# reedrosenbluth/LASS

Hardware: AMD Instinct MI355X
Metric: clips/sec (10s@16kHz) (higher is better)
Workload: dtype f32; 1 GPU; ResUNet30 separate() fp32, batch=16/GPU, 10s@16kHz clips, fixed precomputed condition embedding, seeded random-init weights (BASELINE configs[1]); samples_per_clip=160000, parallelism=clip-sharded x1

## Files before the change

### include/lass_hip.h

```cpp
#ifndef LASS_HIP_H
#define LASS_HIP_H

#include <stddef.h>
#include <stdint.h>

#ifdef __cplusplus
extern "C" {
#endif

typedef struct lass_ctx lass_ctx;

#define LASS_OK 0
#define LASS_ERR_ARG (-1)
#define LASS_ERR_HIP (-2)
#define LASS_ERR_STATE (-3)
#define LASS_ERR_WORKSPACE (-4)

#define LASS_F32 0
#define LASS_I64 1

#define LASS_COMPUTE_F32 0
#define LASS_COMPUTE_BF16 1
#define LASS_COMPUTE_BF16X3 2

int lass_version(void);

int lass_create(lass_ctx** out, int device_id);
int lass_create_multistft(lass_ctx** out, int device_id, int n_fft, int n_windows, const int* win_lengths,
                          int mask_window);
int lass_destroy(lass_ctx* ctx);

const char* lass_last_error(const lass_ctx* ctx);

int lass_set_param(lass_ctx* ctx, const char* name, const void* data, const int64_t* shape, int ndim, int dtype);

int lass_finalize(lass_ctx* ctx, int compute_mode);

int lass_workspace_bytes(const lass_ctx* ctx, int B, int L, size_t* bytes);

int lass_separate(lass_ctx* ctx, const float* mixture, const float* condition, float* out, int B, int L,
                  void* workspace, size_t workspace_bytes, void* stream);

int lass_graph_stats(const lass_ctx* ctx, long* captures, long* replays);
int lass_set_graph_replay(lass_ctx* ctx, int enabled);
int lass_set_wino4_splits(lass_ctx* ctx, int splits);

int lass_separate_components(lass_ctx* ctx, const float* const* mag, const float* cos_mask, const float* sin_mask,
                             const float* condition, float* out, int B, int L, void* workspace, size_t workspace_bytes,
                             void* stream);


int lass_stft_magphase(lass_ctx* ctx, const float* wav, int B, int L, float* mag, float* cos_out, float* sin_out,
                       float* real_out, float* imag_out, void* stream);

int lass_multi_stft(lass_ctx* ctx, const float* wav, int B, int L, int hop, int n_windows, const int* win_lengths,
                    float* const* mag, float* const* cos_out, float* const* sin_out, void* stream);

int lass_stft_components(lass_ctx* ctx, const float* wav, int B, int L, int n_fft, int hop, int n_windows,
                         const int* win_lengths, float* const* mag, float* const* cos_out, float* const* sin_out,
                         void* stream);

int lass_istft(lass_ctx* ctx, const float* real, const float* imag, int B, int T, int L, float* wav,
               float* frames_ws, void* stream);
int lass_istft_nfft(lass_ctx* ctx, const float* real, const float* imag, int B, int T, int L, int n_fft, int win_length,
                    float* wav, void* stream);

int lass_film(lass_ctx* ctx, const float* condition, int B, float* shift, void* stream);
int lass_film_width(const lass_ctx* ctx);
int lass_film_offset(const lass_ctx* ctx, const char* site);
int lass_film_raw(lass_ctx* ctx, const float* condition, int B, float* film, void* stream);

int lass_convblock(lass_ctx* ctx, const char* prefix, const float* x, int B, int H, int W, const float* shift,
                   float* y, float* scratch, void* stream);

int lass_encoder_block(lass_ctx* ctx, const char* name, const float* x, int B, int H, int W, const float* shift, float* y,
                       float* pool, float* scratch, void* stream);

int lass_front_end(lass_ctx* ctx, const float* wav, int B, int L, float* mag, float* cos_out, float* sin_out, float* x0,
                   void* stream);

int lass_workspace_tensor(const lass_ctx* ctx, int B, int L, const char* name, size_t* offset, int64_t shape[4],
                          int64_t strides[4]);

int lass_upconv(lass_ctx* ctx, const char* name, const float* x, int B, int h, int w, const float* shift, float* y,
                void* stream);

int lass_mask_apply(lass_ctx* ctx, const float* x12, const float* mag, const float* cos_in, const float* sin_in,
                    int B, int T, int Tpad, float* out_real, float* out_imag, void* stream);

int lass_sdr_stats(lass_ctx* ctx, const float* ref, const float* est, int B, int L, double* stats, void* stream);

int lass_mix_at_snr(lass_ctx* ctx, float* source, const float* noise, const float* snr_db, float* mixture, int B, int L,
                    double* scratch, void* stream);

#define LASS_WAV_PCM16 0
#define LASS_WAV_PCM32 1
#define LASS_WAV_F32 2
#define LASS_RESAMPLE_MAX_TAPS 16383
#define LASS_RESAMPLE_MAX_TABLE 20480
#define LASS_RESAMPLE_MAX_RATIO 65536
int lass_decode_resample(lass_ctx* ctx, const void* raw, int64_t row_stride_bytes, int B, int frames, int channels, int encoding,
                         int up, int down, const float* taps, int n_taps, float* out, int L_out, void* stream);

int lass_segment_mix(lass_ctx* ctx, const float* waveforms, int B, int L, const int* mix_num, const float* comp_db, int max_comp,
                     const float* noise_db, float* mixture, float* segment, double* scratch, void* stream);


typedef struct lass_text_ctx lass_text_ctx;

int lass_text_create(lass_text_ctx** out, int device_id);
int lass_text_destroy(lass_text_ctx* ctx);
const char* lass_text_last_error(const lass_text_ctx* ctx);
int lass_text_set_param(lass_text_ctx* ctx, const char* name, const void* data, const int64_t* shape, int ndim);
int lass_text_finalize(lass_text_ctx* ctx);
int lass_text_layers(const lass_text_ctx* ctx);
int lass_text_workspace_bytes(const lass_text_ctx* ctx, int N, int S, size_t* bytes);
int lass_text_encode(lass_text_ctx* ctx, const int64_t* input_ids, const int64_t* attention_mask, int N, int S,
                     float* out, float* pooler_out, void* workspace, size_t workspace_bytes, void* stream);


typedef struct lass_audioq_ctx lass_audioq_ctx;

typedef struct lass_audioq_taps {
    float* wave48k;
    float* logmel;
    float* tokens;
    float* stage[4];
    float* embedding;
} lass_audioq_taps;

int lass_audioq_create(lass_audioq_ctx** out, int device_id);
int lass_audioq_destroy(lass_audioq_ctx* ctx);
const char* lass_audioq_last_error(const lass_audioq_ctx* ctx);
int lass_audioq_set_param(lass_audioq_ctx* ctx, const char* name, const void* data, const int64_t* shape, int ndim);
int lass_audioq_finalize(lass_audioq_ctx* ctx);
int lass_audioq_stages(const lass_audioq_ctx* ctx);
int lass_audioq_workspace_bytes(const lass_audioq_ctx* ctx, int B, size_t* bytes);
int lass_audioq_encode_wave48k(lass_audioq_ctx* ctx, const float* wave, const int* lengths, int B, int L, float* out,
                               const lass_audioq_taps* taps, void* workspace, size_t workspace_bytes, void* stream);
int lass_audioq_encode_wave32k(lass_audioq_ctx* ctx, const float* wave, const int* lengths, int B, int L, float* out,
                               const lass_audioq_taps* taps, void* workspace, size_t workspace_bytes, void* stream);


int lass_set_profiling(lass_ctx* ctx, int enabled);
int lass_profile_count(const lass_ctx* ctx);
int lass_profile_get(lass_ctx* ctx, int i, const char** name, double* ms, int* launches);
int lass_profile_reset(lass_ctx* ctx);

#ifdef __cplusplus
}
#endif
#endif
```

### lass_amd/_lib.py

```python
from __future__ import annotations

import ctypes
import os
from ctypes import POINTER, c_char_p, c_double, c_int, c_int64, c_long, c_size_t, c_void_p

_HERE = os.path.dirname(os.path.abspath(__file__))
LIB_PATH = os.environ.get("LASS_HIP_LIB") or os.path.join(_HERE, "csrc", "liblass_hip.so")

_lib = None

SYMBOLS = [
    ("lass_version", c_int, []),
    ("lass_create", c_int, [POINTER(c_void_p), c_int]),
    ("lass_create_multistft", c_int, [POINTER(c_void_p), c_int, c_int, c_int, POINTER(c_int), c_int]),
    ("lass_destroy", c_int, [c_void_p]),
    ("lass_last_error", c_char_p, [c_void_p]),
    ("lass_set_param", c_int, [c_void_p, c_char_p, c_void_p, POINTER(c_int64), c_int, c_int]),
    ("lass_finalize", c_int, [c_void_p, c_int]),
    ("lass_workspace_bytes", c_int, [c_void_p, c_int, c_int, POINTER(c_size_t)]),
    ("lass_separate", c_int, [c_void_p, c_void_p, c_void_p, c_void_p, c_int, c_int, c_void_p, c_size_t, c_void_p]),
    ("lass_stft_magphase", c_int, [c_void_p, c_void_p, c_int, c_int, c_void_p, c_void_p, c_void_p, c_void_p,
                                   c_void_p, c_void_p]),
    ("lass_mix_at_snr", c_int, [c_void_p, c_void_p, c_void_p, c_void_p, c_void_p, c_int, c_int, c_void_p, c_void_p]),
    ("lass_decode_resample", c_int, [c_void_p, c_void_p, c_int64, c_int, c_int, c_int, c_int, c_int, c_int, c_void_p, c_int,
                                     c_void_p, c_int, c_void_p]),
    ("lass_segment_mix", c_int, [c_void_p, c_void_p, c_int, c_int, c_void_p, c_void_p, c_int, c_void_p, c_void_p, c_void_p,
                                 c_void_p, c_void_p]),
    ("lass_multi_stft", c_int, [c_void_p, c_void_p, c_int, c_int, c_int, c_int, POINTER(c_int), POINTER(c_void_p),
                                POINTER(c_void_p), POINTER(c_void_p), c_void_p]),
    ("lass_graph_stats", c_int, [c_void_p, POINTER(c_long), POINTER(c_long)]),
    ("lass_set_graph_replay", c_int, [c_void_p, c_int]),
    ("lass_set_wino4_splits", c_int, [c_void_p, c_int]),
    ("lass_separate_components", c_int, [c_void_p, POINTER(c_void_p), c_void_p, c_void_p, c_void_p, c_void_p, c_int,
                                         c_int, c_void_p, c_size_t, c_void_p]),
    ("lass_stft_components", c_int, [c_void_p, c_void_p, c_int, c_int, c_int, c_int, c_int, POINTER(c_int),
                                     POINTER(c_void_p), POINTER(c_void_p), POINTER(c_void_p), c_void_p]),
    ("lass_istft_nfft", c_int, [c_void_p, c_void_p, c_void_p, c_int, c_int, c_int, c_int, c_int, c_void_p, c_void_p]),
    ("lass_istft", c_int, [c_void_p, c_void_p, c_void_p, c_int, c_int, c_int, c_void_p, c_void_p, c_void_p]),
    ("lass_film", c_int, [c_void_p, c_void_p, c_int, c_void_p, c_void_p]),
    ("lass_film_width", c_int, [c_void_p]),
    ("lass_film_offset", c_int, [c_void_p, c_char_p]),
    ("lass_film_raw", c_int, [c_void_p, c_void_p, c_int, c_void_p, c_void_p]),
    ("lass_convblock", c_int, [c_void_p, c_char_p, c_void_p, c_int, c_int, c_int, c_void_p, c_void_p, c_void_p,
                               c_void_p]),
    ("lass_encoder_block", c_int, [c_void_p, c_char_p, c_void_p, c_int, c_int, c_int, c_void_p, c_void_p, c_void_p,
                                   c_void_p, c_void_p]),
    ("lass_front_end", c_int, [c_void_p, c_void_p, c_int, c_int, c_void_p, c_void_p, c_void_p, c_void_p, c_void_p]),
    ("lass_workspace_tensor", c_int, [c_void_p, c_int, c_int, c_char_p, POINTER(c_size_t), POINTER(c_int64),
                                      POINTER(c_int64)]),
    ("lass_upconv", c_int, [c_void_p, c_char_p, c_void_p, c_int, c_int, c_int, c_void_p, c_void_p, c_void_p]),
    ("lass_mask_apply", c_int, [c_void_p, c_void_p, c_void_p, c_void_p, c_void_p, c_int, c_int, c_int, c_void_p,
                                c_void_p, c_void_p]),
    ("lass_sdr_stats", c_int, [c_void_p, c_void_p, c_void_p, c_int, c_int, c_void_p, c_void_p]),
    ("lass_text_create", c_int, [POINTER(c_void_p), c_int]),
    ("lass_text_destroy", c_int, [c_void_p]),
    ("lass_text_last_error", c_char_p, [c_void_p]),
    ("lass_text_set_param", c_int, [c_void_p, c_char_p, c_void_p, POINTER(c_int64), c_int]),
    ("lass_text_finalize", c_int, [c_void_p]),
    ("lass_text_layers", c_int, [c_void_p]),
    ("lass_text_workspace_bytes", c_int, [c_void_p, c_int, c_int, POINTER(c_size_t)]),
    ("lass_text_encode", c_int, [c_void_p, c_void_p, c_void_p, c_int, c_int, c_void_p, c_void_p, c_void_p, c_size_t,
                                 c_void_p]),
    ("lass_audioq_create", c_int, [POINTER(c_void_p), c_int]),
    ("lass_audioq_destroy", c_int, [c_void_p]),
    ("lass_audioq_last_error", c_char_p, [c_void_p]),
    ("lass_audioq_set_param", c_int, [c_void_p, c_char_p, c_void_p, POINTER(c_int64), c_int]),
    ("lass_audioq_finalize", c_int, [c_void_p]),
    ("lass_audioq_stages", c_int, [c_void_p]),
    ("lass_audioq_workspace_bytes", c_int, [c_void_p, c_int, POINTER(c_size_t)]),
    ("lass_audioq_encode_wave48k", c_int, [c_void_p, c_void_p, POINTER(c_int), c_int, c_int, c_void_p, c_void_p, c_void_p,
                                           c_size_t, c_void_p]),
    ("lass_audioq_encode_wave32k", c_int, [c_void_p, c_void_p, POINTER(c_int), c_int, c_int, c_void_p, c_void_p, c_void_p,
                                           c_size_t, c_void_p]),
    ("lass_set_profiling", c_int, [c_void_p, c_int]),
    ("lass_profile_count", c_int, [c_void_p]),
    ("lass_profile_get", c_int, [c_void_p, c_int, POINTER(c_char_p), POINTER(c_double), POINTER(c_int)]),
    ("lass_profile_reset", c_int, [c_void_p]),
]


class LassError(RuntimeError):
    pass


def load():
    global _lib
    if _lib is not None:
        return _lib
    import torch

    if not os.path.exists(LIB_PATH):
        raise LassError(
            f"{LIB_PATH} is missing - build it with `python -c 'import __graft_entry__ as g; g.build()'` "
            "(hipcc --offload-arch=gfx950).  lass_amd has no CPU fallback.")
    lib = ctypes.CDLL(LIB_PATH, mode=ctypes.RTLD_GLOBAL)
    for name, res, args in SYMBOLS:
        fn = getattr(lib, name)
        fn.restype = res
        fn.argtypes = args
    _lib = lib
    return lib


def check(ctx, rc: int, what: str):
    if rc < 0:
        msg = load().lass_last_error(ctx)
        raise LassError(f"{what} failed ({rc}): {msg.decode() if msg else '?'}")
    return rc
```

### lass_amd/csrc/api.hip

```cpp
#include <hip/hip_runtime.h>

#include <algorithm>
#include <cmath>
#include <cstdio>
#include <cstdlib>
#include <cstring>
#include <map>
#include <string>
#include <vector>

#include "../../include/lass_hip.h"
#include "kernels.h"

namespace {

struct EncSpec { const char* name; int cin, cout, dh, dw; };
struct DecSpec { const char* name; int cin, cout, uh, uw; };
const EncSpec kEnc[7] = {{"encoder_block1", 32, 32, 2, 2},   {"encoder_block2", 32, 64, 2, 2},
                         {"encoder_block3", 64, 128, 2, 2},  {"encoder_block4", 128, 256, 2, 2},
                         {"encoder_block5", 256, 384, 2, 2}, {"encoder_block6", 384, 384, 1, 2},
                         {"conv_block7a", 384, 384, 1, 1}};
const DecSpec kDec[6] = {{"decoder_block1", 384, 384, 1, 2}, {"decoder_block2", 384, 384, 2, 2},
                         {"decoder_block3", 384, 256, 2, 2}, {"decoder_block4", 256, 128, 2, 2},
                         {"decoder_block5", 128, 64, 2, 2},  {"decoder_block6", 64, 32, 2, 2}};
constexpr int kPreCh = 32;
constexpr float kBnEps = 1e-5f;
constexpr int kMaxBranches = LASS_MAX_STFT_WINDOWS;

struct Raw {
    float* d = nullptr;
    std::vector<int64_t> shape;
    size_t n = 0;
};

struct Site {
    std::string film;
    std::string bn;
    int C = 0;
    int off = 0;
};

struct ResBlock {
    std::string prefix;
    int cin = 0, cout = 0;
    int width = 0;
    int s1 = -1, s2 = -1;
    float *w1 = nullptr, *w2 = nullptr, *wsc = nullptr;
    float *u1 = nullptr, *u2 = nullptr, *usc = nullptr;
    float *u1f = nullptr, *u2f = nullptr;
    void *b1 = nullptr, *b2 = nullptr, *bsc16 = nullptr;
    void *b1l = nullptr, *b2l = nullptr, *bscl = nullptr;
    const float* bsc = nullptr;
};

struct ProfEntry {
    const char* name;
    double ms = 0;
    int launches = 0;
};

thread_local std::string g_create_err;

}

struct Geometry {
    int variant = 0;
    int nbr = 1;
    int wins[kMaxBranches] = {1024, 0, 0, 0};
    int nfft = 1024, nbins = 513, fcrop = 512;
    int mask_br = 0;
    int magphase_sem = 0;
};

struct lass_ctx {
    int device = 0;
    std::string err;
    Geometry g;
    EncSpec E[7];
    DecSpec D[6];
    int dec_cat[6] = {0};
    std::string pre_name[kMaxBranches];
    std::map<std::string, Raw> raw;
    bool finalized = false;
    float2* tw2k = nullptr;
    std::vector<Site> sites;
    std::map<std::string, int> site_idx;
    int n_shift = 0;
    float *film_W = nullptr, *film_b = nullptr, *bn_scale = nullptr, *bn_base = nullptr;
    float *bn0_s = nullptr, *bn0_h = nullptr;
    std::vector<ResBlock> enc, dec;
    int dec_site[6] = {0};
    void* up16[6] = {nullptr};
    void* up16l[6] = {nullptr};
    std::vector<void*> owned;
    int compute_mode = LASS_COMPUTE_F32;
    int wino4_mincin = 32;
    int ksplit_force = 0;
    float* stage_part = nullptr;
    size_t stage_part_floats = 0;
    bool fuse_catb = true;
    bool fuse_block = true;
    bool fuse_up = true;
    void* up_sc16 = nullptr;
    bool use_graph = true;
    struct GraphKey {
        const void *mix = nullptr, *cond = nullptr, *out = nullptr, *ws = nullptr;
        int B = 0, L = 0;
        unsigned long gen = 0;
        bool operator==(const GraphKey& o) const {
            return mix == o.mix && cond == o.cond && out == o.out && ws == o.ws && B == o.B && L == o.L && gen == o.gen;
        }
    };
    struct GraphEntry {
        GraphKey key;
        hipGraphExec_t exec = nullptr;
        size_t need = 0;
        int seen = 0;
        unsigned long used = 0;
        bool split = false;
    };
    std::map<std::pair<int, int>, bool> last_split;
    static constexpr int kGraphSlots = 4;
    GraphEntry g_slots[kGraphSlots];
    unsigned long g_tick = 0;
    std::vector<hipGraphExec_t> g_retired;
    hipStream_t g_stream = nullptr;
    int split_batch = 1;
    hipStream_t s2 = nullptr;
    hipEvent_t ev_fork = nullptr, ev_join = nullptr;
    unsigned long gen = 0;
    long g_replays = 0, g_captures = 0;
    bool profiling = false;
    std::vector<ProfEntry> prof;
    std::vector<hipEvent_t> ev_pool;
    struct Pending { int cls; hipEvent_t a, b; };
    std::vector<Pending> pending;
    size_t ev_used = 0;
};

namespace {

#define HIP_TRY(ctx, expr)                                                                                     \
    do {                                                                                                       \
        hipError_t _e = (expr);                                                                                \
        if (_e != hipSuccess) {                                                                                \
            (ctx)->err = std::string(#expr) + ": " + hipGetErrorString(_e);                                     \
            return LASS_ERR_HIP;                                                                               \
        }                                                                                                      \
    } while (0)

int fail(lass_ctx* ctx, int code, const std::string& msg) {
    if (ctx) ctx->err = msg;
    return code;
}

bool starts_with(const std::string& s, const char* p) { return s.rfind(p, 0) == 0; }
bool ends_with(const std::string& s, const char* p) {
    const size_t n = strlen(p);
    return s.size() >= n && s.compare(s.size() - n, n, p) == 0;
}

std::string film_to_bn(const std::string& film) {
    std::string s = "base.";
    for (size_t i = 0; i < film.size(); ++i) {
        if (film[i] == '-' && i + 1 < film.size() && film[i + 1] == '>') {
            s += '.';
            ++i;
        } else {
            s += film[i];
        }
    }
    const size_t p = s.rfind("beta");
    s.replace(p, 4, "bn");
    return s;
}

int add_site(lass_ctx* c, const std::string& film, int C) {
    Site s;
    s.film = film;
    s.bn = film_to_bn(film);
    s.C = C;
    s.off = c->n_shift;
    c->n_shift += C;
    c->site_idx[film] = (int)c->sites.size();
    c->sites.push_back(s);
    return (int)c->sites.size() - 1;
}

const ResBlock& trunk_block(const lass_ctx* c, int i) { return c->enc[c->g.nbr - 1 + i]; }

void build_arch(lass_ctx* c) {
    const Geometry& g = c->g;
    c->sites.clear();
    c->site_idx.clear();
    c->n_shift = 0;
    c->enc.clear();
    c->dec.clear();
    for (int i = 0; i < 7; ++i) c->E[i] = kEnc[i];
    for (int i = 0; i < 6; ++i) c->D[i] = kDec[i];
    c->E[1].cin = kPreCh * g.nbr;
    for (int k = 0; k < g.nbr; ++k) {
        ResBlock rb;
        std::string film;
        if (g.variant == 0) {
            rb.prefix = "base.encoder_block1.conv_block1";
            film = "encoder_block1->conv_block1";
            c->pre_name[k] = "base.pre_conv";
        } else {
            const std::string w = std::to_string(g.wins[k]);
            rb.prefix = "base.encoder_block1s." + w + ".conv_block1";
            film = "encoder_block1s->" + w + "->conv_block1";
            c->pre_name[k] = "base.pre_convs." + w;
        }
        rb.cin = rb.cout = kPreCh;
        rb.width = g.fcrop;
        rb.s1 = add_site(c, film + "->beta1", kPreCh);
        rb.s2 = add_site(c, film + "->beta2", kPreCh);
        c->enc.push_back(rb);
    }
    for (int i = 1; i < 7; ++i) {
        const EncSpec& e = c->E[i];
        ResBlock rb;
        rb.prefix = std::string("base.") + e.name + ".conv_block1";
        rb.cin = e.cin;
        rb.cout = e.cout;
        rb.width = g.fcrop >> i;
        rb.s1 = add_site(c, std::string(e.name) + "->conv_block1->beta1", e.cin);
        rb.s2 = add_site(c, std::string(e.name) + "->conv_block1->beta2", e.cout);
        c->enc.push_back(rb);
    }
    for (int i = 0; i < 6; ++i) {
        const auto& d = c->D[i];
        const int e = 5 - i;
        c->dec_cat[i] = d.cout + c->E[e].cout * (e == 0 ? g.nbr : 1);
        c->dec_site[i] = add_site(c, std::string(d.name) + "->beta1", d.cin);
        ResBlock rb;
        rb.prefix = std::string("base.") + d.name + ".conv_block2";
        rb.cin = c->dec_cat[i];
        rb.cout = d.cout;
        rb.width = g.fcrop >> e;
        rb.s1 = add_site(c, std::string(d.name) + "->conv_block2->beta1", rb.cin);
        rb.s2 = add_site(c, std::string(d.name) + "->conv_block2->beta2", d.cout);
        c->dec.push_back(rb);
    }
}

std::vector<int64_t> expected_shape(const lass_ctx* c, const std::string& name) {
    auto bn_field = [](const std::string& n) {
        return ends_with(n, ".weight") || ends_with(n, ".bias") || ends_with(n, ".running_mean") ||
               ends_with(n, ".running_var");
    };
    if (starts_with(name, "base.bn0.") && bn_field(name)) return {c->g.nbins};
    for (int k = 0; k < c->g.nbr; ++k) {
        if (name == c->pre_name[k] + ".weight") return {kPreCh, 1, 1, 1};
        if (name == c->pre_name[k] + ".bias") return {kPreCh};
    }
    if (name == "base.after_conv.weight") return {3, kPreCh, 1, 1};
    if (name == "base.after_conv.bias") return {3};
    auto res_block = [&](const ResBlock& rb) -> std::vector<int64_t> {
        const std::string& p = rb.prefix;
        if (!starts_with(name, (p + ".").c_str())) return {};
        const std::string f = name.substr(p.size() + 1);
        if (starts_with(f, "bn1.") && bn_field(f)) return {rb.cin};
        if (starts_with(f, "bn2.") && bn_field(f)) return {rb.cout};
        if (f == "conv1.weight") return {rb.cout, rb.cin, 3, 3};
        if (f == "conv2.weight") return {rb.cout, rb.cout, 3, 3};
        if (rb.cin != rb.cout && f == "shortcut.weight") return {rb.cout, rb.cin, 1, 1};
        if (rb.cin != rb.cout && f == "shortcut.bias") return {rb.cout};
        return {};
    };
    for (const auto& rb : c->enc) {
        auto s = res_block(rb);
        if (!s.empty()) return s;
    }
    for (int i = 0; i < 6; ++i) {
        auto s = res_block(c->dec[i]);
        if (!s.empty()) return s;
        const DecSpec& d = c->D[i];
        const std::string p = std::string("base.") + d.name;
        if (name == p + ".conv1.weight") return {d.cin, d.cout, d.uh, d.uw};
        if (starts_with(name, (p + ".bn1.").c_str()) && bn_field(name)) return {d.cin};
    }
    if (starts_with(name, "film.")) {
        for (const auto& s : c->sites) {
            if (name == "film." + s.film + ".weight") return {s.C, LASS_COND};
            if (name == "film." + s.film + ".bias") return {s.C};
        }
    }
    return {};
}

bool ignorable(const std::string& name) {
    if (starts_with(name, "base.stft.") || starts_with(name, "base.istft.")) return true;
    if (ends_with(name, "num_batches_tracked")) return true;
    for (const auto& d : kDec) {
        if (starts_with(name, (std::string("base.") + d.name + ".bn2.").c_str())) return true;
        if (starts_with(name, (std::string("film.") + d.name + "->beta2.").c_str())) return true;
    }
    return false;
}

const float* rawp(const lass_ctx* c, const std::string& name) {
    auto it = c->raw.find(name);
    return it == c->raw.end() ? nullptr : it->second.d;
}

template <typename T>
int dev_alloc(lass_ctx* c, T** p, size_t count) {
    void* v = nullptr;
    HIP_TRY(c, hipMalloc(&v, count * sizeof(T)));
    c->owned.push_back(v);
    *p = (T*)v;
    return 0;
}

void free_owned(lass_ctx* c) {
    for (void* p : c->owned) (void)hipFree(p);
    c->owned.clear();
}

enum ProfClass { P_STFT = 0, P_FILM, P_PRECONV, P_CONV3X3, P_TCONV, P_POOL, P_MASK, P_ISTFT, P_COUNT };
const char* kProfNames[P_COUNT] = {"stft_magphase", "film", "pre_conv", "conv3x3_mfma", "tconv_mfma",
                                   "avg_pool",      "mask_apply", "istft"};

constexpr size_t kProfPairs = 512;

struct ProfScope {
    lass_ctx* c;
    hipStream_t s;
    int cls;
    hipEvent_t b = nullptr;
    bool on = false;
    ProfScope(lass_ctx* ctx, hipStream_t st, int k) : c(ctx), s(st), cls(k) {
        if (!c->profiling || c->ev_used + 2 > c->ev_pool.size()) return;
        hipEvent_t a = c->ev_pool[c->ev_used++];
        b = c->ev_pool[c->ev_used++];
        (void)hipEventRecord(a, s);
        c->pending.push_back({cls, a, b});
        on = true;
    }
    ~ProfScope() {
        if (on) (void)hipEventRecord(b, s);
    }
};

void prof_collect(lass_ctx* c) {
    for (auto& p : c->pending) {
        float ms = 0;
        if (hipEventElapsedTime(&ms, p.a, p.b) == hipSuccess) {
            c->prof[p.cls].ms += ms;
            c->prof[p.cls].launches += 1;
        }
    }
    c->pending.clear();
    c->ev_used = 0;
}

struct CatCopies {
    void* act;
    void* raw;
    int noct;
    const float* scale;
    const float* shift;
};

struct MaskHead {
    const float* mag;
    const float* cosv;
    const float* sinv;
    float* oreal;
    float* oimag;
    int T;
    int nbins;
};

struct PreConv {
    const float* x0;
    const float* w;
    const float* b;
};

struct UpFuse {
    const void* x_act;
    int cin, h, w;
    const void* w16;
    const void* wsc16;
};

struct BlockFusions {
    float* pool_out = nullptr;
    int pool_h = 2;
    long pool_bs = 0;
    int cofs = 0;
    const PreConv* pre = nullptr;
    const MaskHead* head = nullptr;
    const CatCopies* skip_out = nullptr;
    const CatCopies* cat_in = nullptr;
    const Site* act_out = nullptr;
    const CatCopies* pool_copies = nullptr;
    const UpFuse* up = nullptr;
    float* kpart = nullptr;
};

constexpr int kWino4Splits = 4;
int wino4_splits(const lass_ctx* c, const ResBlock& rb, int B, int H, int W) {
    (void)B;
    if (c->compute_mode != LASS_COMPUTE_F32 || c->wino4_mincin <= 0 || !lass_wino4_narrow(H, W) || rb.width % 32 != 16) return 0;
    if (rb.cin < c->wino4_mincin || rb.cout < c->wino4_mincin || rb.cin % 8 != 0 || rb.cout % 32 != 0) return 0;
    return c->ksplit_force ? c->ksplit_force : kWino4Splits;
}
size_t wino4_split_floats(const ResBlock& rb, int S, int B, int H, int W) { return S > 1 ? (size_t)S * B * rb.cout * H * W : 0; }

constexpr int kShortcutGemmMinCin = 256;

int run_resblock(lass_ctx* c, const ResBlock& rb, const float* x, long x_bs, int B, int H, int W, const float* shift,
                 float* a2, float* out, long out_bs, hipStream_t st, const BlockFusions& f = BlockFusions()) {
    const PreConv* pre = f.pre;
    const CatCopies *skip_out = f.skip_out, *cat_in = f.cat_in, *pool_copies = f.pool_copies;
    const float* x0 = pre ? pre->x0 : nullptr;
    const Site& s1 = c->sites[rb.s1];
    const Site& s2 = c->sites[rb.s2];
    const long HW = (long)H * W;
    ConvArgs p;
    p.in = x; p.in_bs = x_bs; p.Cin = rb.cin; p.w = rb.w1; p.Nw = rb.cout; p.N = rb.cout;
    p.pro_scale = c->bn_scale + s1.off; p.pro_shift = shift + s1.off; p.pro_shift_bs = c->n_shift;
    p.epi_scale = c->bn_scale + s2.off; p.epi_shift = shift + s2.off; p.epi_shift_bs = c->n_shift;
    p.out = a2; p.out_bs = rb.cout * HW; p.B = B; p.H = H; p.W = W;
    if (x0) {
        p.in = x0; p.in_bs = HW;
        p.pre_w = pre->w; p.pre_b = pre->b;
    }
    p.w_wino = rb.u1; p.w_wino4 = rb.u1f;
    p.w_bf16 = rb.b1; p.w_bf16_lo = rb.b1l;
    const bool bf1 = c->compute_mode != LASS_COMPUTE_F32 && rb.b1 && rb.b2 && lass_bf16_supported(p) &&
                     (!x0 || W % 32 == 0) && rb.cout % 16 == 0 && (rb.cin == rb.cout || (rb.bsc16 && rb.cin % 16 == 0));
    void* a2_hi = a2;
    void* a2_lo = c->compute_mode == LASS_COMPUTE_BF16X3 ? (void*)((char*)a2 + (size_t)B * rb.cout * HW * 2) : nullptr;
    if (bf1) { p.out_bf16 = a2_hi; p.out_bf16_lo = a2_lo; }
    if ((skip_out || cat_in) && (!bf1 || c->compute_mode != LASS_COMPUTE_BF16))
        return fail(c, LASS_ERR_STATE, "blocked bf16 concat copies need the bf16 kernels");
    if (cat_in) p.in_bf16 = cat_in->act;
    const ConvKind k1 = x0 ? CONV1_ACT_PRE : CONV1_ACT, k2 = x0 ? CONV2_IDENT_PRE : CONV2_IDENT;
    const bool wino1 = !bf1 && rb.u1 && lass_wino_supported(p);
    const int ksplit = bf1 || x0 ? 0 : wino4_splits(c, rb, B, H, W);
    const bool w4_geom = rb.width % 32 == 0 ? !lass_wino4_narrow(H, W) : ksplit > 0;
    if (ksplit > 1) {
        if (!f.kpart) return fail(c, LASS_ERR_STATE, "split-K needs its partial workspace");
        const auto overlaps = [&](const float* a, size_t a_n, const float* b, long b_bs, long b_n) {
            return a < b + (size_t)(B - 1) * b_bs + b_n && b < a + a_n;
        };
        const size_t kn = wino4_split_floats(rb, ksplit, B, H, W);
        if (overlaps(f.kpart, kn, x, x_bs, rb.cin * HW) || overlaps(f.kpart, kn, a2, rb.cout * HW, rb.cout * HW) ||
            overlaps(f.kpart, kn, out, out_bs, rb.cout * HW))
            return fail(c, LASS_ERR_STATE, "the split-K partials must not overlap the block's input, intermediate or output");
    }
    Wino4Split sk;
    if (ksplit > 1) { sk.n = ksplit; sk.part = f.kpart; }
    auto launch_conv1 = [&]() -> int {
        ProfScope ps(c, st, P_CONV3X3);
        if (bf1)
            HIP_TRY(c, lass_launch_conv_bf16(k1, p, st));
        else if (wino1 && rb.u1f && w4_geom && lass_wino4_supported(k1, p, sk))
            HIP_TRY(c, lass_launch_wino4(k1, p, st, sk));
        else if (wino1)
            HIP_TRY(c, lass_launch_wino(k1, p, st));
        else
            HIP_TRY(c, lass_launch_conv(k1, p, st));
        return 0;
    };
    ConvArgs q;
    q.in = a2; q.in_bs = rb.cout * HW; q.Cin = rb.cout; q.w = rb.w2; q.Nw = rb.cout; q.N = rb.cout;
    q.out = out; q.out_bs = out_bs; q.B = B; q.H = H; q.W = W;
    q.pool_out = f.pool_out; q.pool_h = f.pool_h; q.pool_bs = f.pool_bs;
    q.w_wino = rb.u2; q.w2_wino = rb.usc; q.w_wino4 = w4_geom ? rb.u2f : nullptr;
    if (const MaskHead* mh = f.head) {
        q.out = nullptr;
        q.mask_w = rawp(c, "base.after_conv.weight"); q.mask_b = rawp(c, "base.after_conv.bias");
        q.mask_mag = mh->mag; q.mask_cos = mh->cosv; q.mask_sin = mh->sinv;
        q.mask_re = mh->oreal; q.mask_im = mh->oimag; q.mask_T = mh->T; q.mask_nbins = mh->nbins;
    }
    q.w_bf16 = rb.b2; q.w2_bf16 = rb.bsc16; q.w_bf16_lo = rb.b2l; q.w2_bf16_lo = rb.bscl;
    const bool bf2 = bf1;
    if (bf2) { q.in_bf16 = a2_hi; q.in_bf16_lo = a2_lo; }
    if (cat_in) q.in2_bf16 = cat_in->raw;
    if (pool_copies) {
        if (!bf2 || c->compute_mode != LASS_COMPUTE_BF16 || !f.pool_out || f.pool_h != 2)
            return fail(c, LASS_ERR_STATE, "blocked bf16 pooled copies need the bf16 kernels and the fused 2x2 pool");
        q.pool_out = nullptr;
        q.pool_bf16 = pool_copies->raw; q.pool_bf16_act = pool_copies->act;
        q.pool_oct0 = f.cofs / 8; q.pool_noct = pool_copies->noct;
        q.pool_act_scale = pool_copies->scale + f.cofs; q.pool_act_shift = pool_copies->shift + f.cofs; q.act_shift_bs = c->n_shift;
    }
    if (const Site* act_out = f.act_out) {
        if (!bf2 || c->compute_mode != LASS_COMPUTE_BF16) return fail(c, LASS_ERR_STATE, "activated bf16 output needs the bf16 kernels");
        q.out_bf16 = out; q.out = nullptr; q.out_oct0 = 0; q.out_noct = 0;
        q.epi_scale = c->bn_scale + act_out->off; q.epi_shift = shift + act_out->off; q.epi_shift_bs = c->n_shift;
    }
    if (skip_out) {
        q.out = nullptr;
        q.out_bf16 = skip_out->raw; q.out_bf16_act = skip_out->act;
        q.out_oct0 = (rb.cout + f.cofs) / 8; q.out_noct = skip_out->noct;
        q.act_scale = skip_out->scale + rb.cout + f.cofs; q.act_shift = skip_out->shift + rb.cout + f.cofs; q.act_shift_bs = c->n_shift;
    }
    const bool wino2 = !bf2 && rb.u2 && lass_wino_supported(q);
    if (rb.cin == rb.cout) {
        q.res = x; q.res_bs = x_bs;
        if (x0) {
            q.res = x0; q.res_bs = HW;
            q.pre_w = pre->w; q.pre_b = pre->b;
        }
    }
    if (bf2 && x0 && c->fuse_block && c->compute_mode == LASS_COMPUTE_BF16 && skip_out && rb.cin == rb.cout &&
        lass_enc1_fused_bf16_supported(p, q)) {
        ProfScope ps(c, st, P_CONV3X3);
        HIP_TRY(c, lass_launch_enc1_fused_bf16(p, q, st));
        return 0;
    }
    if (rb.cin != rb.cout) { q.in2 = x; q.in2_bs = x_bs; q.Cin2 = rb.cin; q.w2 = rb.wsc; q.bias = rb.bsc; }
    if (const UpFuse* up = f.up) {
        ConvArgs uq;
        uq.in_bf16 = up->x_act; uq.Cin = up->cin; uq.H = up->h; uq.W = up->w; uq.B = B;
        uq.w_bf16 = up->w16; uq.w2_bf16 = up->wsc16;
        if (!(bf2 && !x0 && c->fuse_block && c->compute_mode == LASS_COMPUTE_BF16 && cat_in && f.head && rb.cin != rb.cout &&
              lass_dec6u_fused_bf16_supported(p, q, uq)))
            return fail(c, LASS_ERR_STATE, "decoder_block6 with its transposed conv inside needs the fused bf16 kernel");
        ProfScope ps(c, st, P_CONV3X3);
        HIP_TRY(c, lass_launch_dec6u_fused_bf16(p, q, uq, st));
        return 0;
    }
    if (bf2 && !x0 && c->fuse_block && c->compute_mode == LASS_COMPUTE_BF16 && cat_in && f.head && rb.cin != rb.cout &&
        lass_dec6_fused_bf16_supported(p, q)) {
        ProfScope ps(c, st, P_CONV3X3);
        HIP_TRY(c, lass_launch_dec6_fused_bf16(p, q, st));
        return 0;
    }
    const bool sc_gemm = c->compute_mode == LASS_COMPUTE_F32 && !bf2 && rb.cin != rb.cout && !f.head && rb.cin >= kShortcutGemmMinCin &&
                         wino2 && q.w_wino4 && (ksplit > 0 || lass_wino4_supported(CONV2_SHORTCUT, q)) && lass_pw_gemm_supported(CONV2_SHORTCUT, q);
    if (sc_gemm) {
        const auto overlaps = [&](const float* a, long a_bs, long a_n, const float* b, long b_bs, long b_n) {
            return a < b + (size_t)(B - 1) * b_bs + b_n && b < a + (size_t)(B - 1) * a_bs + a_n;
        };
        if (overlaps(out, out_bs, rb.cout * HW, x, x_bs, rb.cin * HW) || overlaps(out, out_bs, rb.cout * HW, a2, rb.cout * HW, rb.cout * HW))
            return fail(c, LASS_ERR_STATE, "a block's output must not overlap its input or its intermediate");
        ProfScope ps(c, st, P_CONV3X3);
        HIP_TRY(c, lass_launch_pw_gemm(CONV2_SHORTCUT, q, st));
    }
    if (int r1 = launch_conv1()) return r1;
    ProfScope ps(c, st, P_CONV3X3);
    if (sc_gemm) {
        ConvArgs r = q;
        r.in2 = nullptr; r.in2_bs = 0; r.Cin2 = 0; r.w2 = nullptr; r.bias = nullptr;
        r.res = out; r.res_bs = out_bs;
        if (!lass_wino4_supported(CONV2_IDENT, r, sk)) return fail(c, LASS_ERR_STATE, "conv2 with the shortcut as residual");
        HIP_TRY(c, lass_launch_wino4(CONV2_IDENT, r, st, sk));
    } else if (rb.cin == rb.cout) {
        if (bf2)
            HIP_TRY(c, lass_launch_conv_bf16(k2, q, st));
        else if (wino2 && (x0 || ksplit > 0) && q.w_wino4 && lass_wino4_supported(k2, q, sk))
            HIP_TRY(c, lass_launch_wino4(k2, q, st, sk));
        else if (wino2)
            HIP_TRY(c, lass_launch_wino(k2, q, st));
        else
            HIP_TRY(c, lass_launch_conv(k2, q, st));
    } else {
        if (bf2)
            HIP_TRY(c, lass_launch_conv_bf16(CONV2_SHORTCUT, q, st));
        else if (wino2 && q.w_wino4 && lass_wino4_supported(CONV2_SHORTCUT, q))
            HIP_TRY(c, lass_launch_wino4(CONV2_SHORTCUT, q, st));
        else if (wino2)
            HIP_TRY(c, lass_launch_wino(CONV2_SHORTCUT, q, st));
        else
            HIP_TRY(c, lass_launch_conv(CONV2_SHORTCUT, q, st));
    }
    return 0;
}

constexpr int kTconvGemmMinCin = 128;

int run_upconv(lass_ctx* c, int di, const float* x, int B, int h, int w, const float* shift, float* out, long out_bs,
               hipStream_t st, const CatCopies* cb = nullptr, bool x_is_act_bf16 = false) {
    const DecSpec& d = c->D[di];
    const Site& s = c->sites[c->dec_site[di]];
    ConvArgs p;
    p.in = x; p.in_bs = (long)d.cin * h * w; p.Cin = d.cin;
    p.w = rawp(c, std::string("base.") + d.name + ".conv1.weight");
    p.N = p.Nw = d.cout * d.uh * d.uw;
    p.pro_scale = c->bn_scale + s.off; p.pro_shift = shift + s.off; p.pro_shift_bs = c->n_shift;
    p.out = out; p.out_bs = out_bs; p.B = B; p.H = h; p.W = w; p.up_h = d.uh;
    p.w_bf16 = c->up16[di]; p.w_bf16_lo = c->up16l[di];
    if (x_is_act_bf16) {
        if (c->compute_mode != LASS_COMPUTE_BF16 || !p.w_bf16 || !lass_bf16_supported(p))
            return fail(c, LASS_ERR_STATE, "activated bf16 input needs the bf16 kernels");
        p.in_bf16 = x;
    }
    if (cb) {
        if (c->compute_mode != LASS_COMPUTE_BF16 || !p.w_bf16 || !lass_bf16_supported(p))
            return fail(c, LASS_ERR_STATE, "blocked bf16 concat copies need the bf16 kernels");
        p.out = nullptr;
        p.out_bf16 = cb->raw; p.out_bf16_act = cb->act; p.out_oct0 = 0; p.out_noct = cb->noct;
        p.act_scale = cb->scale; p.act_shift = cb->shift; p.act_shift_bs = c->n_shift;
    }
    ProfScope ps(c, st, P_TCONV);
    if (c->compute_mode != LASS_COMPUTE_F32 && p.w_bf16 && lass_bf16_supported(p))
        HIP_TRY(c, lass_launch_conv_bf16(TCONV_ACT, p, st));
    else if (c->compute_mode == LASS_COMPUTE_F32 && d.cin >= kTconvGemmMinCin && lass_pw_gemm_supported(TCONV_ACT, p))
        HIP_TRY(c, lass_launch_pw_gemm(TCONV_ACT, p, st));
    else
        HIP_TRY(c, lass_launch_conv(TCONV_ACT, p, st));
    return 0;
}

struct Plan {
    int B, L, T, Tp;
    size_t total = 0;
    size_t mag, cosv, sinv, x0[kMaxBranches], shift, a2, cat[6], pool[6], center, decout[6], oreal, oimag;
    size_t kpart = 0;
    bool has_kpart = false;
    int eh[7], ew[7];
};

size_t bump(size_t& total, size_t floats) {
    const size_t off = total;
    total += (floats * sizeof(float) + 255) / 256 * 256;
    return off;
}

int make_plan(const lass_ctx* c, int B, int L, Plan* pl) {
    const Geometry& g = c->g;
    if (B <= 0 || L <= g.nfft / 2) return LASS_ERR_ARG;
    pl->B = B; pl->L = L;
    pl->T = 1 + L / LASS_HOP;
    pl->Tp = (pl->T + 31) / 32 * 32;
    const size_t clip_max = (size_t)c->dec_cat[5] * pl->Tp * g.fcrop * sizeof(float);
    if (clip_max > 0xFFFF0000ull) return LASS_ERR_ARG;
    size_t& t = pl->total;
    t = 0;
    const size_t spec = (size_t)B * pl->T * g.nbins;
    pl->mag = bump(t, spec); pl->cosv = bump(t, spec); pl->sinv = bump(t, spec);
    for (int k = 0; k < g.nbr; ++k) pl->x0[k] = bump(t, (size_t)B * pl->Tp * g.fcrop);
    pl->shift = bump(t, (size_t)B * c->n_shift);
    int h = pl->Tp, w = g.fcrop;
    size_t a2max = 0;
    for (int i = 0; i < 7; ++i) {
        pl->eh[i] = h; pl->ew[i] = w;
        const size_t o = (size_t)B * c->E[i].cout * h * w;
        if (o > a2max) a2max = o;
        h /= c->E[i].dh; w /= c->E[i].dw;
        if (i < 6) pl->pool[i] = bump(t, (size_t)B * c->E[i].cout * (i == 0 ? g.nbr : 1) * h * w);
    }
    pl->center = bump(t, (size_t)B * c->E[6].cout * pl->eh[6] * pl->ew[6]);
    for (int d = 0; d < 6; ++d) {
        const int e = 5 - d;
        const size_t hw = (size_t)pl->eh[e] * pl->ew[e];
        pl->cat[d] = bump(t, (size_t)B * c->dec_cat[d] * hw);
        pl->decout[d] = bump(t, (size_t)B * c->D[d].cout * hw);
    }
    pl->a2 = bump(t, a2max);
    pl->oreal = bump(t, spec); pl->oimag = bump(t, spec);
    size_t kmax = 0;
    for (int i = 1; i < 7; ++i) {
        const ResBlock& rb = trunk_block(c, i);
        kmax = std::max(kmax, wino4_split_floats(rb, wino4_splits(c, rb, B, pl->eh[i], pl->ew[i]), B, pl->eh[i], pl->ew[i]));
    }
    for (int d = 0; d < 6; ++d) {
        const ResBlock& rb = c->dec[d];
        kmax = std::max(kmax, wino4_split_floats(rb, wino4_splits(c, rb, B, pl->eh[5 - d], pl->ew[5 - d]), B, pl->eh[5 - d], pl->ew[5 - d]));
    }
    pl->has_kpart = kmax > 0;
    if (kmax) pl->kpart = bump(t, kmax);
    return 0;
}

int use_device(lass_ctx* c) {
    if (!c) return LASS_ERR_ARG;
    HIP_TRY(c, hipSetDevice(c->device));
    return 0;
}

int check_ready(lass_ctx* c) {
    if (!c) return LASS_ERR_ARG;
    if (!c->finalized) return fail(c, LASS_ERR_STATE, "lass_finalize has not been called (or a parameter changed since)");
    return use_device(c);
}

void drop_graphs(lass_ctx* c) {
    for (auto& e : c->g_slots) {
        if (e.exec) (void)hipGraphExecDestroy(e.exec);
        e = lass_ctx::GraphEntry();
    }
    for (hipGraphExec_t x : c->g_retired) (void)hipGraphExecDestroy(x);
    c->g_retired.clear();
}

bool split_halves(const lass_ctx* c, int B) { return c->split_batch > 0 && !c->profiling && B >= 8 && (B % 2) == 0; }

int stage_kpart(lass_ctx* c, const ResBlock& rb, int B, int H, int W, BlockFusions* f) {
    const size_t need = wino4_split_floats(rb, wino4_splits(c, rb, B, H, W), B, H, W);
    if (need > c->stage_part_floats) {
        if (c->stage_part) HIP_TRY(c, hipFree(c->stage_part));
        c->stage_part = nullptr;
        c->stage_part_floats = 0;
        HIP_TRY(c, hipMalloc((void**)&c->stage_part, need * sizeof(float)));
        c->stage_part_floats = need;
    }
    if (need) f->kpart = c->stage_part;
    return 0;
}

const ResBlock* find_block(const lass_ctx* c, const std::string& prefix) {
    for (const auto& rb : c->enc) if (rb.prefix == prefix) return &rb;
    for (const auto& rb : c->dec) if (rb.prefix == prefix) return &rb;
    return nullptr;
}

}

extern "C" {

int lass_version(void) { return 10300; }

const char* lass_last_error(const lass_ctx* ctx) { return ctx ? ctx->err.c_str() : g_create_err.c_str(); }

static int create_impl(lass_ctx** out, int device_id, const Geometry& geom) {
    if (!out) return LASS_ERR_ARG;
    *out = nullptr;
    int ndev = 0;
    hipError_t e = hipGetDeviceCount(&ndev);
    if (e != hipSuccess || ndev <= 0) {
        g_create_err = std::string("no HIP device available: ") + hipGetErrorString(e) +
                       " (liblass_hip has no CPU fallback)";
        return LASS_ERR_HIP;
    }
    if (device_id < 0 || device_id >= ndev) {
        g_create_err = "device_id out of range";
        return LASS_ERR_ARG;
    }
    hipDeviceProp_t prop;
    e = hipGetDeviceProperties(&prop, device_id);
    if (e != hipSuccess) {
        g_create_err = std::string("hipGetDeviceProperties: ") + hipGetErrorString(e);
        return LASS_ERR_HIP;
    }
    if (std::string(prop.gcnArchName).rfind("gfx950", 0) != 0) {
        g_create_err = std::string("device is ") + prop.gcnArchName + "; liblass_hip is built for gfx950 only";
        return LASS_ERR_HIP;
    }
    lass_ctx* c = new lass_ctx();
    c->device = device_id;
    c->g = geom;
    if (const char* e = getenv("LASS_FUSE_CATB")) c->fuse_catb = atoi(e) != 0;
    if (const char* e = getenv("LASS_FUSE_BLOCK")) c->fuse_block = atoi(e) != 0;
    if (const char* e = getenv("LASS_FUSE_UP")) c->fuse_up = atoi(e) != 0;
    if (const char* e = getenv("LASS_WINO4")) c->wino4_mincin = atoi(e);
    if (const char* e = getenv("LASS_SPLIT")) c->split_batch = std::max(0, std::min(2, atoi(e)));
    if (const char* e = getenv("LASS_GRAPH")) c->use_graph = atoi(e) != 0;
    c->prof.resize(P_COUNT);
    for (int i = 0; i < P_COUNT; ++i) c->prof[i].name = kProfNames[i];
    build_arch(c);
    if (hipSetDevice(device_id) != hipSuccess) {
        g_create_err = "hipSetDevice failed";
        delete c;
        return LASS_ERR_HIP;
    }
    std::vector<float2> tw2k(2048);
    for (int k = 0; k < 2048; ++k) {
        const double a = 2.0 * M_PI * k / 2048.0;
        tw2k[k] = make_float2((float)std::cos(a), (float)std::sin(a));
    }
    if (hipMalloc((void**)&c->tw2k, sizeof(float2) * 2048) != hipSuccess ||
        hipMemcpy(c->tw2k, tw2k.data(), sizeof(float2) * 2048, hipMemcpyHostToDevice) != hipSuccess) {
        g_create_err = "allocating FFT tables failed";
        delete c;
        return LASS_ERR_HIP;
    }
    *out = c;
    return 0;
}

int lass_create(lass_ctx** out, int device_id) { return create_impl(out, device_id, Geometry()); }

int lass_create_multistft(lass_ctx** out, int device_id, int n_fft, int n_windows, const int* win_lengths,
                          int mask_window) {
    if (!out) return LASS_ERR_ARG;
    *out = nullptr;
    Geometry g;
    g.variant = 1;
    g.magphase_sem = 1;
    if (n_fft != 2048 || n_windows < 1 || n_windows > kMaxBranches || !win_lengths) {
        g_create_err = "lass_create_multistft: n_fft must be 2048 and 1 <= n_windows <= 4";
        return LASS_ERR_ARG;
    }
    g.nfft = n_fft; g.nbins = n_fft / 2 + 1; g.fcrop = n_fft / 2; g.nbr = n_windows; g.mask_br = -1;
    for (int k = 0; k < n_windows; ++k) {
        const int w = win_lengths[k];
        if (w < 32 || w > n_fft || (2048 % w) != 0) {
            g_create_err = "lass_create_multistft: window lengths must be powers of two in [32, n_fft]";
            return LASS_ERR_ARG;
        }
        for (int j = 0; j < k; ++j)
            if (g.wins[j] == w) {
                g_create_err = "lass_create_multistft: duplicate window length";
                return LASS_ERR_ARG;
            }
        g.wins[k] = w;
        if (w == mask_window) g.mask_br = k;
    }
    if (g.mask_br < 0) {
        g_create_err = "lass_create_multistft: mask_window is not one of the analysis windows";
        return LASS_ERR_ARG;
    }
    return create_impl(out, device_id, g);
}

int lass_destroy(lass_ctx* c) {
    if (!c) return LASS_ERR_ARG;
    (void)hipSetDevice(c->device);
    free_owned(c);
    for (auto& kv : c->raw) (void)hipFree(kv.second.d);
    for (auto e : c->ev_pool) (void)hipEventDestroy(e);
    (void)hipDeviceSynchronize();
    drop_graphs(c);
    if (c->g_stream) (void)hipStreamDestroy(c->g_stream);
    if (c->s2) (void)hipStreamDestroy(c->s2);
    if (c->ev_join) (void)hipEventDestroy(c->ev_join);
    if (c->ev_fork) (void)hipEventDestroy(c->ev_fork);
    (void)hipFree(c->tw2k);
    (void)hipFree(c->stage_part);
    delete c;
    return 0;
}

int lass_set_param(lass_ctx* c, const char* name_c, const void* data, const int64_t* shape, int ndim, int dtype) {
    if (!c || !name_c || !data || ndim < 0 || (ndim > 0 && !shape)) return fail(c, LASS_ERR_ARG, "bad argument");
    const std::string name(name_c);
    std::vector<int64_t> want = expected_shape(c, name);
    if (want.empty()) {
        if (ignorable(name)) return 1;
        return fail(c, LASS_ERR_ARG, "unknown parameter '" + name + "'");
    }
    if (dtype != LASS_F32) return fail(c, LASS_ERR_ARG, "parameter '" + name + "' must be float32");
    std::vector<int64_t> got(shape, shape + ndim);
    if (got != want) {
        std::string m = "shape mismatch for '" + name + "': got (";
        for (auto v : got) m += std::to_string(v) + ",";
        m += ") want (";
        for (auto v : want) m += std::to_string(v) + ",";
        return fail(c, LASS_ERR_ARG, m + ")");
    }
    size_t n = 1;
    for (auto v : want) n *= (size_t)v;
    HIP_TRY(c, hipSetDevice(c->device));
    Raw& r = c->raw[name];
    if (!r.d) HIP_TRY(c, hipMalloc((void**)&r.d, n * sizeof(float)));
    r.shape = want;
    r.n = n;
    HIP_TRY(c, hipMemcpy(r.d, data, n * sizeof(float), hipMemcpyDefault));
    c->finalized = false;
    return 0;
}

int lass_finalize(lass_ctx* c, int compute_mode) {
    if (!c) return LASS_ERR_ARG;
    if (compute_mode != LASS_COMPUTE_F32 && compute_mode != LASS_COMPUTE_BF16 && compute_mode != LASS_COMPUTE_BF16X3)
        return fail(c, LASS_ERR_ARG, "unsupported compute mode");
    c->last_split.clear();
    c->compute_mode = compute_mode;
    HIP_TRY(c, hipSetDevice(c->device));
    HIP_TRY(c, hipDeviceSynchronize());
    drop_graphs(c);
    free_owned(c);
    c->finalized = false;
    hipStream_t st = nullptr;
    auto need = [&](const std::string& n) -> const float* {
        const float* p = rawp(c, n);
        if (!p && c->err.empty()) c->err = "missing parameter '" + n + "'";
        return p;
    };
    c->err.clear();
    if (dev_alloc(c, &c->bn_scale, c->n_shift) || dev_alloc(c, &c->bn_base, c->n_shift) ||
        dev_alloc(c, &c->film_W, (size_t)c->n_shift * LASS_COND) || dev_alloc(c, &c->film_b, c->n_shift) ||
        dev_alloc(c, &c->bn0_s, c->g.nbins) || dev_alloc(c, &c->bn0_h, c->g.nbins))
        return LASS_ERR_HIP;
    for (const auto& s : c->sites) {
        const float *g = need(s.bn + ".weight"), *b = need(s.bn + ".bias"), *m = need(s.bn + ".running_mean"),
                    *v = need(s.bn + ".running_var"), *fw = need("film." + s.film + ".weight"),
                    *fb = need("film." + s.film + ".bias");
        if (!g || !b || !m || !v || !fw || !fb) return LASS_ERR_STATE;
        HIP_TRY(c, lass_launch_bnfold(g, b, m, v, s.C, kBnEps, c->bn_scale + s.off, c->bn_base + s.off, st));
        HIP_TRY(c, hipMemcpyAsync(c->film_W + (size_t)s.off * LASS_COND, fw, (size_t)s.C * LASS_COND * sizeof(float),
                                  hipMemcpyDeviceToDevice, st));
        HIP_TRY(c, hipMemcpyAsync(c->film_b + s.off, fb, s.C * sizeof(float), hipMemcpyDeviceToDevice, st));
    }
    {
        const float *g = need("base.bn0.weight"), *b = need("base.bn0.bias"), *m = need("base.bn0.running_mean"),
                    *v = need("base.bn0.running_var");
        if (!g || !b || !m || !v) return LASS_ERR_STATE;
        HIP_TRY(c, lass_launch_bnfold(g, b, m, v, c->g.nbins, kBnEps, c->bn0_s, c->bn0_h, st));
    }
    for (int k = 0; k < c->g.nbr; ++k)
        if (!need(c->pre_name[k] + ".weight") || !need(c->pre_name[k] + ".bias")) return LASS_ERR_STATE;
    if (!need("base.after_conv.weight") || !need("base.after_conv.bias")) return LASS_ERR_STATE;
    auto prep = [&](ResBlock& rb) -> int {
        const float *w1 = need(rb.prefix + ".conv1.weight"), *w2 = need(rb.prefix + ".conv2.weight");
        if (!w1 || !w2) return LASS_ERR_STATE;
        if (dev_alloc(c, &rb.w1, (size_t)rb.cout * rb.cin * 9) || dev_alloc(c, &rb.w2, (size_t)rb.cout * rb.cout * 9))
            return LASS_ERR_HIP;
        HIP_TRY(c, lass_launch_relayout_conv(w1, rb.cout, rb.cin, 9, rb.w1, st));
        HIP_TRY(c, lass_launch_relayout_conv(w2, rb.cout, rb.cout, 9, rb.w2, st));
        rb.u1 = rb.u2 = rb.usc = nullptr;
        rb.u1f = rb.u2f = nullptr;
        rb.b1 = rb.b2 = rb.bsc16 = rb.b1l = rb.b2l = rb.bscl = nullptr;
        const bool bfm = c->compute_mode == LASS_COMPUTE_BF16 || c->compute_mode == LASS_COMPUTE_BF16X3;
        const bool split = c->compute_mode == LASS_COMPUTE_BF16X3;
        if (bfm && rb.cin % 16 == 0 && rb.cout % 16 == 0) {
            unsigned short *t1 = nullptr, *t2 = nullptr;
            if (dev_alloc(c, &t1, (size_t)rb.cout * rb.cin * 9) || dev_alloc(c, &t2, (size_t)rb.cout * rb.cout * 9))
                return LASS_ERR_HIP;
            HIP_TRY(c, lass_launch_weights_bf16(w1, rb.cout, rb.cin, 9, t1, 0, 0, st));
            HIP_TRY(c, lass_launch_weights_bf16(w2, rb.cout, rb.cout, 9, t2, 0, 0, st));
            rb.b1 = t1; rb.b2 = t2;
            if (split) {
                unsigned short *l1 = nullptr, *l2 = nullptr;
                if (dev_alloc(c, &l1, (size_t)rb.cout * rb.cin * 9) || dev_alloc(c, &l2, (size_t)rb.cout * rb.cout * 9))
                    return LASS_ERR_HIP;
                HIP_TRY(c, lass_launch_weights_bf16(w1, rb.cout, rb.cin, 9, l1, 1, 0, st));
                HIP_TRY(c, lass_launch_weights_bf16(w2, rb.cout, rb.cout, 9, l2, 1, 0, st));
                rb.b1l = l1; rb.b2l = l2;
            }
        }
        if (c->compute_mode == LASS_COMPUTE_F32) {
            if (dev_alloc(c, &rb.u1, (size_t)16 * rb.cout * rb.cin) || dev_alloc(c, &rb.u2, (size_t)16 * rb.cout * rb.cout))
                return LASS_ERR_HIP;
            HIP_TRY(c, lass_launch_wino_weights(w1, rb.cout, rb.cin, rb.u1, st));
            HIP_TRY(c, lass_launch_wino_weights(w2, rb.cout, rb.cout, rb.u2, st));
            const bool w4_level = rb.width % 32 == 0, w4_narrow = rb.width % 32 == 16;
            if ((w4_level || w4_narrow) && c->wino4_mincin > 0 && rb.cin >= c->wino4_mincin && rb.cin % 8 == 0 && rb.cout % 32 == 0) {
                if (dev_alloc(c, &rb.u1f, (size_t)36 * rb.cout * rb.cin)) return LASS_ERR_HIP;
                HIP_TRY(c, lass_launch_wino4_weights(w1, rb.cout, rb.cin, rb.u1f, st));
            }
            if (c->wino4_mincin > 0 && rb.cout >= c->wino4_mincin && rb.cout % 32 == 0 && rb.cin % 8 == 0 &&
                (w4_level ? rb.cin != rb.cout || rb.cout == kPreCh : w4_narrow && rb.cin >= c->wino4_mincin)) {
                if (dev_alloc(c, &rb.u2f, (size_t)36 * rb.cout * rb.cout)) return LASS_ERR_HIP;
                HIP_TRY(c, lass_launch_wino4_weights(w2, rb.cout, rb.cout, rb.u2f, st));
            }
        }
        rb.wsc = nullptr;
        rb.bsc = nullptr;
        if (rb.cin != rb.cout) {
            const float *ws = need(rb.prefix + ".shortcut.weight"), *bs = need(rb.prefix + ".shortcut.bias");
            if (!ws || !bs) return LASS_ERR_STATE;
            if (dev_alloc(c, &rb.wsc, (size_t)rb.cout * rb.cin)) return LASS_ERR_HIP;
            HIP_TRY(c, lass_launch_relayout_conv(ws, rb.cout, rb.cin, 1, rb.wsc, st));
            rb.bsc = bs;
            if (bfm && rb.b1) {
                unsigned short* t3 = nullptr;
                if (dev_alloc(c, &t3, (size_t)rb.cout * rb.cin)) return LASS_ERR_HIP;
                HIP_TRY(c, lass_launch_weights_bf16(ws, rb.cout, rb.cin, 1, t3, 0, 0, st));
                rb.bsc16 = t3;
                if (split) {
                    unsigned short* l3 = nullptr;
                    if (dev_alloc(c, &l3, (size_t)rb.cout * rb.cin)) return LASS_ERR_HIP;
                    HIP_TRY(c, lass_launch_weights_bf16(ws, rb.cout, rb.cin, 1, l3, 1, 0, st));
                    rb.bscl = l3;
                }
            }
            if (c->compute_mode == LASS_COMPUTE_F32) {
                if (dev_alloc(c, &rb.usc, (size_t)4 * rb.cout * rb.cin)) return LASS_ERR_HIP;
                HIP_TRY(c, lass_launch_wino_shortcut_weights(ws, rb.cout, rb.cin, rb.usc, st));
            }
        }
        return 0;
    };
    for (auto& rb : c->enc) { int r = prep(rb); if (r) return r; }
    for (auto& rb : c->dec) { int r = prep(rb); if (r) return r; }
    for (int i = 0; i < 6; ++i) {
        const auto& d = c->D[i];
        const float* wu = need(std::string("base.") + d.name + ".conv1.weight");
        if (!wu) return LASS_ERR_STATE;
        c->up16[i] = c->up16l[i] = nullptr;
        if (c->compute_mode != LASS_COMPUTE_F32 && d.cin % 16 == 0) {
            const int N = d.cout * d.uh * d.uw;
            unsigned short *t = nullptr, *l = nullptr;
            if (dev_alloc(c, &t, (size_t)N * d.cin)) return LASS_ERR_HIP;
            HIP_TRY(c, lass_launch_weights_bf16(wu, N, d.cin, 1, t, 0, 1, st));
            c->up16[i] = t;
            if (c->compute_mode == LASS_COMPUTE_BF16X3) {
                if (dev_alloc(c, &l, (size_t)N * d.cin)) return LASS_ERR_HIP;
                HIP_TRY(c, lass_launch_weights_bf16(wu, N, d.cin, 1, l, 1, 1, st));
                c->up16l[i] = l;
            }
        }
    }
    c->up_sc16 = nullptr;
    {
        const DecSpec& d = c->D[5];
        const ResBlock& rb = c->dec[5];
        if (c->compute_mode == LASS_COMPUTE_BF16 && c->g.variant == 0 && d.cin == 64 && d.cout == 32 && d.uh == 2 && d.uw == 2 &&
            rb.cin == 64 && rb.cout == 32 && c->up16[5]) {
            const float* wu = need(std::string("base.") + d.name + ".conv1.weight");
            const float* ws = need(rb.prefix + ".shortcut.weight");
            if (!wu || !ws) return LASS_ERR_STATE;
            float* tmp = nullptr;
            unsigned short* t16 = nullptr;
            if (dev_alloc(c, &tmp, (size_t)4 * rb.cout * d.cin) || dev_alloc(c, &t16, (size_t)4 * rb.cout * d.cin)) return LASS_ERR_HIP;
            HIP_TRY(c, lass_launch_compose_up_shortcut(ws, wu, d.cin, d.cout, rb.cin, rb.cout, tmp, st));
            HIP_TRY(c, lass_launch_weights_bf16(tmp, 4 * rb.cout, d.cin, 1, t16, 0, 0, st));
            c->up_sc16 = t16;
        }
    }
    HIP_TRY(c, hipStreamSynchronize(st));
    c->finalized = true;
    ++c->gen;
    return 0;
}

int lass_workspace_bytes(const lass_ctx* c, int B, int L, size_t* bytes) {
    if (!c || !bytes) return LASS_ERR_ARG;
    Plan pl;
    if (make_plan(c, B, L, &pl)) return LASS_ERR_ARG;
    *bytes = pl.total;
    if (split_halves(c, B)) {
        Plan ph;
        if (make_plan(c, B / 2, L, &ph)) return LASS_ERR_ARG;
        const size_t both = 2 * ((ph.total + 255) / 256 * 256);
        if (both > *bytes) *bytes = both;
    }
    return 0;
}

int lass_film_width(const lass_ctx* c) { return c ? c->n_shift : LASS_ERR_ARG; }

int lass_film_offset(const lass_ctx* c, const char* site) {
    if (!c || !site) return -1;
    auto it = c->site_idx.find(site);
    return it == c->site_idx.end() ? -1 : c->sites[it->second].off;
}

int lass_film(lass_ctx* c, const float* cond, int B, float* shift, void* stream) {
    int r = check_ready(c);
    if (r) return r;
    if (!cond || !shift || B <= 0) return fail(c, LASS_ERR_ARG, "lass_film: bad argument");
    HIP_TRY(c, lass_launch_film(cond, B, c->film_W, c->film_b, c->bn_base, c->n_shift, shift, (hipStream_t)stream));
    return 0;
}

int lass_film_raw(lass_ctx* c, const float* cond, int B, float* film, void* stream) {
    int r = check_ready(c);
    if (r) return r;
    if (!cond || !film || B <= 0) return fail(c, LASS_ERR_ARG, "lass_film_raw: bad argument");
    HIP_TRY(c, lass_launch_film(cond, B, c->film_W, c->film_b, nullptr, c->n_shift, film, (hipStream_t)stream));
    return 0;
}

int lass_stft_magphase(lass_ctx* c, const float* wav, int B, int L, float* mag, float* cos_out, float* sin_out,
                       float* real_out, float* imag_out, void* stream) {
    if (!c || !wav || B <= 0 || L <= LASS_NFFT / 2) return fail(c, LASS_ERR_ARG, "lass_stft_magphase: bad argument");
    if (int r = use_device(c)) return r;
    const int T = 1 + L / LASS_HOP;
    StftBranch br;
    br.wlen = LASS_NFFT; br.mag = mag; br.cosv = cos_out; br.sinv = sin_out; br.real = real_out; br.imag = imag_out;
    HIP_TRY(c, lass_launch_stft2(wav, B, L, LASS_NFFT, LASS_HOP, T, T, 1, &br, 0, nullptr, nullptr, c->tw2k,
                                 (hipStream_t)stream));
    return 0;
}

int lass_stft_components(lass_ctx* c, const float* wav, int B, int L, int n_fft, int hop, int n_windows,
                         const int* win_lengths, float* const* mag, float* const* cos_out, float* const* sin_out,
                         void* stream) {
    if (!c || !wav || !win_lengths || !mag || !cos_out || !sin_out || B <= 0 || hop <= 0 || n_windows <= 0 ||
        n_windows > LASS_MAX_STFT_WINDOWS || (n_fft != 1024 && n_fft != 2048) || L <= n_fft / 2)
        return fail(c, LASS_ERR_ARG, "lass_stft_components: bad argument (n_fft 1024 or 2048, at most 4 windows, L > n_fft/2)");
    StftBranch br[LASS_MAX_STFT_WINDOWS];
    for (int i = 0; i < n_windows; ++i) {
        const int w = win_lengths[i];
        if (w < 32 || w > n_fft || (2048 % w) != 0)
            return fail(c, LASS_ERR_ARG, "lass_stft_components: window lengths must be powers of two in [32, n_fft]");
        if (!mag[i] || !cos_out[i] || !sin_out[i]) return fail(c, LASS_ERR_ARG, "lass_stft_components: null output");
        br[i].wlen = w; br[i].mag = mag[i]; br[i].cosv = cos_out[i]; br[i].sinv = sin_out[i];
    }
    if (int r = use_device(c)) return r;
    const int T = 1 + L / hop;
    HIP_TRY(c, lass_launch_stft2(wav, B, L, n_fft, hop, T, T, n_windows, br, 1, nullptr, nullptr, c->tw2k,
                                 (hipStream_t)stream));
    return 0;
}

int lass_multi_stft(lass_ctx* c, const float* wav, int B, int L, int hop, int n_windows, const int* win_lengths,
                    float* const* mag, float* const* cos_out, float* const* sin_out, void* stream) {
    if (!c || !wav || !win_lengths || !mag || !cos_out || !sin_out || B <= 0 || hop <= 0 || n_windows <= 0 ||
        n_windows > LASS_MAX_STFT_WINDOWS)
        return fail(c, LASS_ERR_ARG, "lass_multi_stft: bad argument");
    for (int i = 0; i < n_windows; ++i) {
        const int N = win_lengths[i];
        if (N != 256 && N != 512 && N != 1024 && N != 2048)
            return fail(c, LASS_ERR_ARG, "lass_multi_stft: window lengths must be 256, 512, 1024 or 2048");
        if (L <= N / 2) return fail(c, LASS_ERR_ARG, "lass_multi_stft: waveform shorter than the reflect padding");
        if (!mag[i] || !cos_out[i] || !sin_out[i]) return fail(c, LASS_ERR_ARG, "lass_multi_stft: null output");
    }
    if (int r = use_device(c)) return r;
    HIP_TRY(c, lass_launch_multi_stft(wav, B, L, hop, n_windows, win_lengths, c->tw2k, mag, cos_out, sin_out,
                                      (hipStream_t)stream));
    return 0;
}

int lass_istft(lass_ctx* c, const float* real, const float* imag, int B, int T, int L, float* wav, float* frames_ws,
               void* stream) {
    (void)frames_ws;
    return lass_istft_nfft(c, real, imag, B, T, L, LASS_NFFT, LASS_NFFT, wav, stream);
}

int lass_istft_nfft(lass_ctx* c, const float* real, const float* imag, int B, int T, int L, int n_fft, int win_length,
                    float* wav, void* stream) {
    if (!c || !real || !imag || !wav || B <= 0 || T <= 0 || L <= 0 || (n_fft != 1024 && n_fft != 2048) ||
        win_length < 32 || win_length > n_fft || (2048 % win_length) != 0 ||
        (long)L + n_fft / 2 > (long)(T - 1) * LASS_HOP + n_fft)
        return fail(c, LASS_ERR_ARG, "lass_istft: bad argument");
    if (int r = use_device(c)) return r;
    HIP_TRY(c, lass_launch_istft2(real, imag, B, T, L, n_fft, win_length, LASS_HOP, c->tw2k, wav, (hipStream_t)stream));
    return 0;
}

int lass_convblock(lass_ctx* c, const char* prefix, const float* x, int B, int H, int W, const float* shift, float* y,
                   float* scratch, void* stream) {
    int r = check_ready(c);
    if (r) return r;
    if (!prefix || !x || !shift || !y || !scratch) return fail(c, LASS_ERR_ARG, "lass_convblock: bad argument");
    const ResBlock* rb = find_block(c, prefix);
    if (!rb) return fail(c, LASS_ERR_ARG, std::string("lass_convblock: unknown block '") + prefix + "'");
    const long HW = (long)H * W;
    BlockFusions f;
    if ((r = stage_kpart(c, *rb, B, H, W, &f))) return r;
    return run_resblock(c, *rb, x, rb->cin * HW, B, H, W, shift, scratch, y, rb->cout * HW, (hipStream_t)stream, f);
}

int lass_encoder_block(lass_ctx* c, const char* name, const float* x, int B, int H, int W, const float* shift, float* y,
                       float* pool, float* scratch, void* stream) {
    int r = check_ready(c);
    if (r) return r;
    if (!name || !x || !shift || !y || !scratch || B <= 0 || H <= 0 || W <= 0)
        return fail(c, LASS_ERR_ARG, "lass_encoder_block: bad argument");
    for (size_t bi = 0; bi < c->enc.size(); ++bi) {
        const ResBlock& rb = c->enc[bi];
        if (rb.prefix != std::string(name) + ".conv_block1") continue;
        const EncSpec& e = c->E[bi < (size_t)c->g.nbr ? 0 : bi - c->g.nbr + 1];
        const long HW = (long)H * W;
        const bool pooled = e.dw == 2;
        if (pooled && (!pool || W % 2 != 0)) return fail(c, LASS_ERR_ARG, "lass_encoder_block: pool output needed, W even");
        const bool fuse = pooled && (H % e.dh) == 0;
        hipStream_t st = (hipStream_t)stream;
        BlockFusions f;
        if (fuse) { f.pool_out = pool; f.pool_h = e.dh; }
        if ((r = stage_kpart(c, rb, B, H, W, &f))) return r;
        r = run_resblock(c, rb, x, rb.cin * HW, B, H, W, shift, scratch, y, rb.cout * HW, st, f);
        if (r) return r;
        if (pooled && !fuse) HIP_TRY(c, lass_launch_pool(y, rb.cout * HW, B, rb.cout, H, W, e.dh, e.dw, pool, st));
        return 0;
    }
    return fail(c, LASS_ERR_ARG, std::string("lass_encoder_block: unknown encoder '") + name + "'");
}

int lass_front_end(lass_ctx* c, const float* wav, int B, int L, float* mag, float* cos_out, float* sin_out, float* x0,
                   void* stream) {
    int r = check_ready(c);
    if (r) return r;
    const Geometry& g = c->g;
    if (!wav || !x0 || B <= 0 || L <= g.nfft / 2) return fail(c, LASS_ERR_ARG, "lass_front_end: bad argument");
    const int T = 1 + L / LASS_HOP, Tp = (T + 31) / 32 * 32;
    StftBranch br[kMaxBranches];
    for (int k = 0; k < g.nbr; ++k) {
        br[k].wlen = g.wins[k];
        br[k].x0 = x0 + (size_t)k * B * Tp * g.fcrop;
        if (k == g.mask_br) { br[k].mag = mag; br[k].cosv = cos_out; br[k].sinv = sin_out; }
    }
    HIP_TRY(c, lass_launch_stft2(wav, B, L, g.nfft, LASS_HOP, T, Tp, g.nbr, br, g.magphase_sem, c->bn0_s, c->bn0_h,
                                 c->tw2k, (hipStream_t)stream));
    return 0;
}

int lass_workspace_tensor(const lass_ctx* c, int B, int L, const char* name_c, size_t* offset, int64_t shape[4],
                          int64_t strides[4]) {
    if (!c || !name_c || !offset || !shape || !strides) return LASS_ERR_ARG;
    if (auto it = c->last_split.find({B, L}); it != c->last_split.end() && it->second) return LASS_ERR_STATE;
    Plan pl;
    if (make_plan(c, B, L, &pl)) return LASS_ERR_ARG;
    const Geometry& g = c->g;
    const std::string name(name_c);
    auto put = [&](size_t off, int64_t C, int64_t H, int64_t W, int64_t bs) {
        *offset = off;
        shape[0] = B; shape[1] = C; shape[2] = H; shape[3] = W;
        strides[0] = bs; strides[1] = H * W; strides[2] = W; strides[3] = 1;
        return 0;
    };
    const int64_t spec = (int64_t)pl.T * g.nbins;
    if (name == "mag") return put(pl.mag, 1, pl.T, g.nbins, spec);
    if (name == "cos") return put(pl.cosv, 1, pl.T, g.nbins, spec);
    if (name == "sin") return put(pl.sinv, 1, pl.T, g.nbins, spec);
    if (name == "out_real") return put(pl.oreal, 1, pl.T, g.nbins, spec);
    if (name == "out_imag") return put(pl.oimag, 1, pl.T, g.nbins, spec);
    for (int k = 0; k < g.nbr; ++k)
        if (name == (g.variant == 0 ? std::string("x0") : "x0." + std::to_string(g.wins[k])))
            return put(pl.x0[k], 1, pl.Tp, g.fcrop, (int64_t)pl.Tp * g.fcrop);
    for (int i = 0; i < 7; ++i) {
        const EncSpec& e = c->E[i];
        const int64_t H = pl.eh[i], W = pl.ew[i];
        const int64_t C = (int64_t)e.cout * (i == 0 ? g.nbr : 1);
        if (name == e.name) {
            if (i == 6) return put(pl.center, C, H, W, C * H * W);
            const int d = 5 - i;
            return put(pl.cat[d] + (size_t)c->D[d].cout * H * W * sizeof(float), C, H, W, (int64_t)c->dec_cat[d] * H * W);
        }
        if (i < 6 && name == std::string(e.name) + ".pool")
            return put(pl.pool[i], C, H / e.dh, W / e.dw, C * (H / e.dh) * (W / e.dw));
    }
    for (int d = 0; d < 6; ++d) {
        const int64_t H = pl.eh[5 - d], W = pl.ew[5 - d], C = c->D[d].cout;
        if (name == std::string(c->D[d].name) + ".up") return put(pl.cat[d], C, H, W, (int64_t)c->dec_cat[d] * H * W);
        if (name == c->D[d].name) return put(pl.decout[d], C, H, W, C * H * W);
    }
    return LASS_ERR_ARG;
}

int lass_upconv(lass_ctx* c, const char* name, const float* x, int B, int h, int w, const float* shift, float* y,
                void* stream) {
    int r = check_ready(c);
    if (r) return r;
    if (!name || !x || !shift || !y) return fail(c, LASS_ERR_ARG, "lass_upconv: bad argument");
    for (int i = 0; i < 6; ++i)
        if (std::string("base.") + c->D[i].name == name)
            return run_upconv(c, i, x, B, h, w, shift, y, (long)c->D[i].cout * h * c->D[i].uh * w * c->D[i].uw,
                              (hipStream_t)stream);
    return fail(c, LASS_ERR_ARG, std::string("lass_upconv: unknown decoder '") + name + "'");
}

int lass_mask_apply(lass_ctx* c, const float* x12, const float* mag, const float* cos_in, const float* sin_in, int B,
                    int T, int Tpad, float* out_real, float* out_imag, void* stream) {
    int r = check_ready(c);
    if (r) return r;
    if (!x12 || !mag || !cos_in || !sin_in || !out_real || !out_imag)
        return fail(c, LASS_ERR_ARG, "lass_mask_apply: bad argument");
    HIP_TRY(c, lass_launch_mask(x12, rawp(c, "base.after_conv.weight"), rawp(c, "base.after_conv.bias"), mag, cos_in,
                                sin_in, B, T, Tpad, c->g.fcrop, out_real, out_imag, (hipStream_t)stream));
    return 0;
}

int lass_sdr_stats(lass_ctx* c, const float* ref, const float* est, int B, int L, double* stats, void* stream) {
    if (!c || !ref || !est || !stats || B <= 0 || L <= 0) return fail(c, LASS_ERR_ARG, "lass_sdr_stats: bad argument");
    if (int r = use_device(c)) return r;
    HIP_TRY(c, lass_launch_sdr(ref, est, B, L, stats, (hipStream_t)stream));
    return 0;
}

int lass_mix_at_snr(lass_ctx* c, float* source, const float* noise, const float* snr_db, float* mixture, int B, int L,
                    double* scratch, void* stream) {
    if (!c || !source || !noise || !snr_db || !mixture || !scratch || B <= 0 || L <= 0)
        return fail(c, LASS_ERR_ARG, "lass_mix_at_snr: bad argument");
    if (int r = use_device(c)) return r;
    HIP_TRY(c, lass_launch_mix_at_snr(source, noise, snr_db, mixture, B, L, scratch, (hipStream_t)stream));
    return 0;
}

int lass_decode_resample(lass_ctx* c, const void* raw, int64_t row_stride_bytes, int B, int frames, int channels, int encoding,
                         int up, int down, const float* taps, int n_taps, float* out, int L_out, void* stream) {
    const char* w = "lass_decode_resample: ";
    if (!c) return LASS_ERR_ARG;
    if (!raw || !out || B <= 0 || B > 65535 || frames <= 0) return fail(c, LASS_ERR_ARG, std::string(w) + "raw, out non-NULL, 1 <= B <= 65535, frames >= 1");
    if (encoding != LASS_WAV_PCM16 && encoding != LASS_WAV_PCM32 && encoding != LASS_WAV_F32)
        return fail(c, LASS_ERR_ARG, std::string(w) + "encoding must be LASS_WAV_PCM16, LASS_WAV_PCM32 or LASS_WAV_F32");
    if (channels < 1 || channels > 8) return fail(c, LASS_ERR_ARG, std::string(w) + "1 ... 8 channels");
    if (up < 1 || down < 1 || up > LASS_RESAMPLE_MAX_RATIO || down > LASS_RESAMPLE_MAX_RATIO)
        return fail(c, LASS_ERR_ARG, std::string(w) + "up and down must lie in 1 ... " + std::to_string(LASS_RESAMPLE_MAX_RATIO));
    const bool fir = up != 1 || down != 1;
    if (fir) {
        if (!taps || n_taps < 1 || n_taps % 2 == 0) return fail(c, LASS_ERR_ARG, std::string(w) + "taps non-NULL, n_taps odd");
        if (n_taps > LASS_RESAMPLE_MAX_TAPS)
            return fail(c, LASS_ERR_ARG, std::string(w) + std::to_string(n_taps) + " taps exceed the cap of " +
                        std::to_string(LASS_RESAMPLE_MAX_TAPS) + " (resample on the host)");
        if (lass_resample_table_floats(up, n_taps) > LASS_RESAMPLE_MAX_TABLE)
            return fail(c, LASS_ERR_ARG, std::string(w) + "the polyphase table up * (ceil(n_taps/up) | 1) exceeds " +
                        std::to_string(LASS_RESAMPLE_MAX_TABLE) + " floats");
    }
    const long long want = ((long long)frames * up + down - 1) / down;
    if (L_out <= 0 || want != (long long)L_out)
        return fail(c, LASS_ERR_ARG, std::string(w) + "L_out must be ceil(frames*up/down) = " + std::to_string(want));
    const long long row_bytes = (long long)frames * channels * (encoding == LASS_WAV_PCM16 ? 2 : 4);
    if (row_stride_bytes < row_bytes || row_stride_bytes % 4 != 0)
        return fail(c, LASS_ERR_ARG, std::string(w) + "row_stride_bytes must be a multiple of 4 and hold a row (" +
                    std::to_string(row_bytes) + " bytes)");
    if (reinterpret_cast<uintptr_t>(raw) % 4 != 0) return fail(c, LASS_ERR_ARG, std::string(w) + "raw must be 4-byte aligned");
    if (int r = use_device(c)) return r;
    HIP_TRY(c, lass_launch_decode_resample(raw, row_stride_bytes, B, frames, channels, encoding, up, down, taps, n_taps, out, L_out,
                                           (hipStream_t)stream));
    return 0;
}

int lass_segment_mix(lass_ctx* c, const float* waveforms, int B, int L, const int* mix_num, const float* comp_db, int max_comp,
                     const float* noise_db, float* mixture, float* segment, double* scratch, void* stream) {
    if (!c || !waveforms || !mix_num || !comp_db || !noise_db || !mixture || !segment || !scratch || B <= 0 || L <= 0)
        return fail(c, LASS_ERR_ARG, "lass_segment_mix: bad argument");
    if (max_comp < 1 || max_comp > 7) return fail(c, LASS_ERR_ARG, "lass_segment_mix: max_comp (max_mix_num - 1) must be 1 ... 7");
    if (mixture == waveforms || segment == waveforms || mixture == segment)
        return fail(c, LASS_ERR_ARG, "lass_segment_mix: waveforms, mixture and segment must be three different buffers");
    if (int r = use_device(c)) return r;
    HIP_TRY(c, lass_launch_segment_mix(waveforms, B, L, mix_num, comp_db, max_comp, noise_db, mixture, segment, scratch,
                                       (hipStream_t)stream));
    return 0;
}

struct Components {
    const float* mag[kMaxBranches];
    const float* cosv;
    const float* sinv;
};

static int separate_impl(lass_ctx* c, const float* mixture, const Components* comp, const float* condition, float* out,
                         int B, int L, void* workspace, size_t workspace_bytes, void* stream, const char* who) {
    int r = check_ready(c);
    if (r) return r;
    const Geometry& g = c->g;
    if ((!mixture && !comp) || !condition || !out || !workspace) return fail(c, LASS_ERR_ARG, std::string(who) + ": null pointer");
    Plan pl;
    if (make_plan(c, B, L, &pl))
        return fail(c, LASS_ERR_ARG, std::string(who) + ": need B >= 1 and " + std::to_string(g.nfft / 2) +
                                         " < L, with decoder_block6's concat (" + std::to_string(c->dec_cat[5]) +
                                         " ch x frames x " + std::to_string(g.fcrop) +
                                         " bins, f32) below 4 GiB per clip (longer clips: ResUNet30.chunk_inference)");
    if (workspace_bytes < pl.total)
        return fail(c, LASS_ERR_WORKSPACE, "workspace too small: need " + std::to_string(pl.total) + " bytes");
    if (((uintptr_t)workspace & 255) != 0) return fail(c, LASS_ERR_ARG, "workspace must be 256-byte aligned");
    hipStream_t st = (hipStream_t)stream;
    char* ws = (char*)workspace;
    auto F = [&](size_t off) { return (float*)(ws + off); };
    const int T = pl.T, Tp = pl.Tp, nbr = g.nbr;
    float* shift = F(pl.shift);
    const float *mag_m = F(pl.mag), *cos_m = F(pl.cosv), *sin_m = F(pl.sinv);
    if (mixture) {
        ProfScope ps(c, st, P_STFT);
        StftBranch br[kMaxBranches];
        for (int k = 0; k < nbr; ++k) {
            br[k].wlen = g.wins[k];
            br[k].x0 = F(pl.x0[k]);
            if (k == g.mask_br) { br[k].mag = F(pl.mag); br[k].cosv = F(pl.cosv); br[k].sinv = F(pl.sinv); }
        }
        HIP_TRY(c, lass_launch_stft2(mixture, B, L, g.nfft, LASS_HOP, T, Tp, nbr, br, g.magphase_sem, c->bn0_s, c->bn0_h,
                                     c->tw2k, st));
    } else {
        ProfScope ps(c, st, P_STFT);
        for (int k = 0; k < nbr; ++k) {
            if (!comp->mag[k]) return fail(c, LASS_ERR_ARG, std::string(who) + ": null magnitude");
            HIP_TRY(c, lass_launch_x0_from_mag(comp->mag[k], B, T, Tp, g.fcrop, c->bn0_s, c->bn0_h, F(pl.x0[k]), st));
        }
        if (!comp->cosv || !comp->sinv) return fail(c, LASS_ERR_ARG, std::string(who) + ": null phase");
        mag_m = comp->mag[g.mask_br]; cos_m = comp->cosv; sin_m = comp->sinv;
    }
    {
        ProfScope ps(c, st, P_FILM);
        HIP_TRY(c, lass_launch_film(condition, B, c->film_W, c->film_b, c->bn_base, c->n_shift, shift, st));
    }
    CatCopies cb[6];
    bool use_cb[6] = {false, false, false, false, false, false};
    for (int d = 1; d < 6; ++d) {
        const int e = 5 - d;
        const ResBlock& rd = c->dec[d];
        const ResBlock& re = c->enc[nbr - 1 + e];
        const long hw = (long)pl.eh[e] * pl.ew[e];
        use_cb[d] = c->fuse_catb && c->compute_mode == LASS_COMPUTE_BF16 && c->D[d].uh == 2 && c->D[d].uw == 2 &&
                    rd.cout % 16 == 0 && rd.b1 && rd.b2 && rd.bsc16 && c->up16[d] && re.b1 && re.b2;
        cb[d].act = F(pl.cat[d]);
        cb[d].raw = (char*)F(pl.cat[d]) + (size_t)B * rd.cin * hw * 2;
        cb[d].noct = rd.cin / 8;
        cb[d].scale = c->bn_scale + c->sites[rd.s1].off;
        cb[d].shift = shift + c->sites[rd.s1].off;
    }
    CatCopies pc[4];
    bool use_pc[4] = {false, false, false, false};
    for (int i = 0; i < 4; ++i) {
        const ResBlock& nx = c->enc[nbr - 1 + i + 1];
        const long hwo = (long)pl.eh[i + 1] * pl.ew[i + 1];
        use_pc[i] = c->fuse_catb && c->compute_mode == LASS_COMPUTE_BF16 && c->E[i].dh == 2 && pl.ew[i] % 32 == 0 &&
                    use_cb[5 - i] && use_cb[5 - (i + 1)] && nx.cin != nx.cout && nx.cin % 16 == 0 && nx.b1 && nx.b2 && nx.bsc16;
        pc[i].act = F(pl.pool[i]);
        pc[i].raw = (char*)F(pl.pool[i]) + (size_t)B * nx.cin * hwo * 2;
        pc[i].noct = nx.cin / 8;
        pc[i].scale = c->bn_scale + c->sites[nx.s1].off;
        pc[i].shift = shift + c->sites[nx.s1].off;
    }
    const float* x = nullptr;
    for (int i = 0; i < 7; ++i) {
        const int H = pl.eh[i], W = pl.ew[i];
        const long HW = (long)H * W;
        const EncSpec& e = c->E[i];
        const int nb = i == 0 ? nbr : 1;
        float* o = nullptr;
        long o_bs = 0;
        for (int k = 0; k < nb; ++k) {
            const ResBlock& rb = c->enc[i == 0 ? k : nbr - 1 + i];
            BlockFusions f;
            f.cofs = k * e.cout;
            if (i < 6) {
                const int d = 5 - i;
                o = F(pl.cat[d]) + (size_t)(c->D[d].cout + f.cofs) * HW;
                o_bs = (long)c->dec_cat[d] * HW;
                const long Ho = H / e.dh, Wo = W / e.dw;
                f.pool_out = F(pl.pool[i]) + (size_t)f.cofs * Ho * Wo;
                f.pool_h = e.dh;
                f.pool_bs = (long)e.cout * nb * Ho * Wo;
            } else {
                o = F(pl.center);
                o_bs = rb.cout * HW;
            }
            PreConv pre{};
            if (i == 0) {
                pre = PreConv{F(pl.x0[k]), rawp(c, c->pre_name[k] + ".weight"), rawp(c, c->pre_name[k] + ".bias")};
                f.pre = &pre;
            }
            if (i < 5 && use_cb[5 - i]) f.skip_out = &cb[5 - i];
            if (i >= 1 && i <= 4 && use_pc[i - 1]) f.cat_in = &pc[i - 1];
            if (i < 4 && use_pc[i]) f.pool_copies = &pc[i];
            if (pl.has_kpart) f.kpart = F(pl.kpart);
            r = run_resblock(c, rb, x, rb.cin * HW, B, H, W, shift, F(pl.a2), o, o_bs, st, f);
            if (r) return r;
        }
        x = i < 6 ? F(pl.pool[i]) : o;
    }
    bool x_act = false;
    for (int d = 0; d < 6; ++d) {
        const int e = 5 - d;
        const int H = pl.eh[e], W = pl.ew[e];
        const long HW = (long)H * W;
        const int h = H / c->D[d].uh, w = W / c->D[d].uw;
        const ResBlock& rb = c->dec[d];
        BlockFusions f;
        const UpFuse upf{x, c->D[d].cin, h, w, c->up16[d], c->up_sc16};
        const bool fuse_up = d == 5 && c->fuse_up && c->fuse_block && use_cb[d] && x_act && c->up_sc16 &&
                             c->compute_mode == LASS_COMPUTE_BF16 && rb.cout == 32 && rb.cin == 64 && W == g.fcrop && W % 32 == 0 &&
                             H % 2 == 0 && (unsigned long long)H * W * 8ull < 0x10000000ull;
        if (fuse_up) {
            f.up = &upf;
        } else {
            r = run_upconv(c, d, x, B, h, w, shift, F(pl.cat[d]), rb.cin * HW, st, use_cb[d] ? &cb[d] : nullptr, x_act);
            if (r) return r;
        }
        x_act = d < 5 && c->fuse_catb && c->compute_mode == LASS_COMPUTE_BF16 && rb.b1 && rb.b2 && rb.bsc16 &&
                rb.cout % 16 == 0 && c->up16[d + 1];
        if (x_act) f.act_out = &c->sites[c->dec_site[d + 1]];
        if (use_cb[d]) f.cat_in = &cb[d];
        const MaskHead head{mag_m, cos_m, sin_m, F(pl.oreal), F(pl.oimag), T, g.nbins};
        if (d == 5) f.head = &head;
        if (pl.has_kpart) f.kpart = F(pl.kpart);
        r = run_resblock(c, rb, F(pl.cat[d]), rb.cin * HW, B, H, W, shift, F(pl.a2), F(pl.decout[d]), rb.cout * HW, st, f);
        if (r) return r;
        x = F(pl.decout[d]);
    }
    {
        ProfScope ps(c, st, P_ISTFT);
        HIP_TRY(c, lass_launch_istft2(F(pl.oreal), F(pl.oimag), B, T, L, g.nfft, g.wins[g.mask_br], LASS_HOP, c->tw2k, out, st));
    }
    return 0;
}

static int separate_any(lass_ctx* c, const float* mixture, const float* condition, float* out, int B, int L, void* workspace,
                        size_t workspace_bytes, hipStream_t stream, bool capturing) {
    Plan ph;
    if (!c->finalized || !split_halves(c, B) || !mixture || !condition || !out || !workspace || (!capturing && c->split_batch < 2) ||
        make_plan(c, B / 2, L, &ph) || 2 * ((ph.total + 255) / 256 * 256) > workspace_bytes) {
        c->last_split[{B, L}] = false;
        return separate_impl(c, mixture, nullptr, condition, out, B, L, workspace, workspace_bytes, stream, "lass_separate");
    }
    c->last_split[{B, L}] = true;
    HIP_TRY(c, hipSetDevice(c->device));
    if (!c->ev_fork) HIP_TRY(c, hipEventCreateWithFlags(&c->ev_fork, hipEventDisableTiming));
    if (!c->s2) {
        HIP_TRY(c, hipStreamCreateWithFlags(&c->s2, hipStreamNonBlocking));
        HIP_TRY(c, hipEventCreateWithFlags(&c->ev_join, hipEventDisableTiming));
    }
    const int h = B / 2;
    const size_t half_ws = (ph.total + 255) / 256 * 256;
    HIP_TRY(c, hipEventRecord(c->ev_fork, stream));
    HIP_TRY(c, hipStreamWaitEvent(c->s2, c->ev_fork, 0));
    int r = separate_impl(c, mixture, nullptr, condition, out, h, L, workspace, half_ws, stream, "lass_separate");
    const int r2 = separate_impl(c, mixture + (size_t)h * L, nullptr, condition + (size_t)h * LASS_COND, out + (size_t)h * L, h, L,
                                 (char*)workspace + half_ws, half_ws, c->s2, "lass_separate");
    if (!r) r = r2;
    HIP_TRY(c, hipEventRecord(c->ev_join, c->s2));
    HIP_TRY(c, hipStreamWaitEvent(stream, c->ev_join, 0));
    return r;
}

int lass_separate(lass_ctx* c, const float* mixture, const float* condition, float* out, int B, int L, void* workspace,
                  size_t workspace_bytes, void* stream) {
    if (!c) return LASS_ERR_ARG;
    if (!mixture) return fail(c, LASS_ERR_ARG, "lass_separate: null pointer");
    lass_ctx::GraphKey key;
    key.mix = mixture; key.cond = condition; key.out = out; key.ws = workspace; key.B = B; key.L = L; key.gen = c->gen;
    if (c->use_graph && !c->profiling && c->finalized) {
        ++c->g_tick;
        lass_ctx::GraphEntry* slot = nullptr;
        for (auto& e : c->g_slots)
            if (e.seen > 0 && e.key == key) slot = &e;
        if (!slot) {
            for (auto& e : c->g_slots)
                if (!slot || (!e.exec && slot->exec) || (!e.exec == !slot->exec && e.used < slot->used)) slot = &e;
            if (slot->exec) {
                c->g_retired.push_back(slot->exec);
                if (c->g_retired.size() > 8) {
                    HIP_TRY(c, hipSetDevice(c->device));
                    HIP_TRY(c, hipDeviceSynchronize());
                    for (hipGraphExec_t x : c->g_retired) (void)hipGraphExecDestroy(x);
                    c->g_retired.clear();
                }
            }
            *slot = lass_ctx::GraphEntry();
            slot->key = key;
        }
        slot->used = c->g_tick;
        ++slot->seen;
        if (slot->exec) {
            if (workspace_bytes < slot->need)
                return fail(c, LASS_ERR_WORKSPACE, "workspace too small: need " + std::to_string(slot->need) + " bytes");
            HIP_TRY(c, hipSetDevice(c->device));
            HIP_TRY(c, hipGraphLaunch(slot->exec, (hipStream_t)stream));
            ++c->g_replays;
            c->last_split[{B, L}] = slot->split;
            return 0;
        }
        if (slot->seen >= 3) {
            {
                int r0 = check_ready(c);
                if (r0) return r0;
                Plan pl0;
                if (!condition || !out || !workspace || make_plan(c, B, L, &pl0) || workspace_bytes < pl0.total ||
                    ((uintptr_t)workspace & 255) != 0)
                    return separate_any(c, mixture, condition, out, B, L, workspace, workspace_bytes, (hipStream_t)stream, false);
                slot->need = pl0.total;
                if (split_halves(c, B)) {
                    Plan ph0;
                    if (!make_plan(c, B / 2, L, &ph0) && 2 * ((ph0.total + 255) / 256 * 256) <= workspace_bytes)
                        slot->need = std::max(slot->need, 2 * ((ph0.total + 255) / 256 * 256));
                }
            }
            HIP_TRY(c, hipSetDevice(c->device));
            if (!c->g_stream) HIP_TRY(c, hipStreamCreateWithFlags(&c->g_stream, hipStreamNonBlocking));
            bool ok = false;
            if (hipStreamBeginCapture(c->g_stream, hipStreamCaptureModeThreadLocal) == hipSuccess) {
                const int r = separate_any(c, mixture, condition, out, B, L, workspace, workspace_bytes, c->g_stream, true);
                hipGraph_t graph = nullptr;
                const hipError_t e = hipStreamEndCapture(c->g_stream, &graph);
                if (r == 0 && e == hipSuccess && graph && hipGraphInstantiate(&slot->exec, graph, nullptr, nullptr, 0) == hipSuccess) {
                    ok = true;
                    if (auto it = c->last_split.find({B, L}); it != c->last_split.end()) slot->split = it->second;
                } else {
                    slot->exec = nullptr;
                }
                if (graph) (void)hipGraphDestroy(graph);
            }
            if (ok) {
                ++c->g_captures;
                HIP_TRY(c, hipGraphLaunch(slot->exec, (hipStream_t)stream));
                return 0;
            }
            (void)hipGetLastError();
            c->use_graph = false;
            c->err.clear();
        }
    }
    return separate_any(c, mixture, condition, out, B, L, workspace, workspace_bytes, (hipStream_t)stream, false);
}

int lass_set_graph_replay(lass_ctx* c, int enabled) {
    if (!c) return LASS_ERR_ARG;
    c->use_graph = enabled != 0;
    return 0;
}

int lass_set_wino4_splits(lass_ctx* c, int splits) {
    if (!c || (splits != 0 && splits != 1 && splits != 2 && splits != 4)) return fail(c, LASS_ERR_ARG, "lass_set_wino4_splits: 0, 1, 2 or 4");
    c->ksplit_force = splits;
    ++c->gen;
    return 0;
}

int lass_graph_stats(const lass_ctx* c, long* captures, long* replays) {
    if (!c) return LASS_ERR_ARG;
    if (captures) *captures = c->g_captures;
    if (replays) *replays = c->g_replays;
    return c->use_graph ? 1 : 0;
}

int lass_separate_components(lass_ctx* c, const float* const* mag, const float* cos_mask, const float* sin_mask,
                             const float* condition, float* out, int B, int L, void* workspace, size_t workspace_bytes,
                             void* stream) {
    if (!c) return LASS_ERR_ARG;
    if (!mag || !cos_mask || !sin_mask) return fail(c, LASS_ERR_ARG, "lass_separate_components: null pointer");
    Components comp;
    for (int k = 0; k < kMaxBranches; ++k) comp.mag[k] = k < c->g.nbr ? mag[k] : nullptr;
    comp.cosv = cos_mask; comp.sinv = sin_mask;
    return separate_impl(c, nullptr, &comp, condition, out, B, L, workspace, workspace_bytes, stream,
                         "lass_separate_components");
}

int lass_set_profiling(lass_ctx* c, int enabled) {
    if (!c) return LASS_ERR_ARG;
    if (enabled && c->ev_pool.size() < 2 * kProfPairs) {
        HIP_TRY(c, hipSetDevice(c->device));
        c->pending.reserve(kProfPairs);
        while (c->ev_pool.size() < 2 * kProfPairs) {
            hipEvent_t e;
            HIP_TRY(c, hipEventCreate(&e));
            c->ev_pool.push_back(e);
        }
    }
    c->profiling = enabled != 0;
    return 0;
}
int lass_profile_count(const lass_ctx* c) { return c ? P_COUNT : LASS_ERR_ARG; }
int lass_profile_get(lass_ctx* c, int i, const char** name, double* ms, int* launches) {
    if (!c || i < 0 || i >= P_COUNT) return LASS_ERR_ARG;
    prof_collect(c);
    if (name) *name = c->prof[i].name;
    if (ms) *ms = c->prof[i].ms;
    if (launches) *launches = c->prof[i].launches;
    return 0;
}
int lass_profile_reset(lass_ctx* c) {
    if (!c) return LASS_ERR_ARG;
    prof_collect(c);
    for (auto& p : c->prof) { p.ms = 0; p.launches = 0; }
    return 0;
}

}
```

### lass_amd/csrc/kernels.h

```cpp
#pragma once
#include <hip/hip_runtime.h>
#include <stddef.h>
#include <stdint.h>

constexpr int LASS_NFFT = 1024;
constexpr int LASS_HOP = 160;
constexpr int LASS_NBINS = 513;
constexpr int LASS_FCROP = 512;
constexpr int LASS_COND = 512;
constexpr int LASS_MAX_STFT_WINDOWS = 4;

struct ConvArgs {
    const float* in = nullptr;
    long in_bs = 0;
    int Cin = 0;
    const float* w = nullptr;
    int Nw = 0;
    const float* pro_scale = nullptr;
    const float* pro_shift = nullptr;
    int pro_shift_bs = 0;
    const float* in2 = nullptr;
    long in2_bs = 0;
    int Cin2 = 0;
    const float* w2 = nullptr;
    const float* bias = nullptr;
    const float* res = nullptr;
    long res_bs = 0;
    const float* epi_scale = nullptr;
    const float* epi_shift = nullptr;
    int epi_shift_bs = 0;
    float* out = nullptr;
    long out_bs = 0;
    int B = 0, H = 0, W = 0;
    int N = 0;
    int up_h = 1;
    const float* w_wino = nullptr;
    const float* w2_wino = nullptr;
    const float* w_wino4 = nullptr;
    const void* w_bf16 = nullptr;
    const void* w2_bf16 = nullptr;
    const void* w_bf16_lo = nullptr;
    const void* w2_bf16_lo = nullptr;
    void* out_bf16 = nullptr;
    void* out_bf16_lo = nullptr;
    const void* in_bf16 = nullptr;
    const void* in_bf16_lo = nullptr;
    void* out_bf16_act = nullptr;
    const float* act_scale = nullptr;
    const float* act_shift = nullptr;
    int act_shift_bs = 0;
    int out_oct0 = 0;
    int out_noct = 0;
    const void* in2_bf16 = nullptr;
    void* pool_bf16 = nullptr;
    void* pool_bf16_act = nullptr;
    int pool_oct0 = 0;
    int pool_noct = 0;
    const float* pool_act_scale = nullptr;
    const float* pool_act_shift = nullptr;
    const float* pre_w = nullptr;
    const float* pre_b = nullptr;
    const float* mask_w = nullptr;
    const float* mask_b = nullptr;
    const float* mask_mag = nullptr;
    const float* mask_cos = nullptr;
    const float* mask_sin = nullptr;
    float* mask_re = nullptr;
    float* mask_im = nullptr;
    int mask_T = 0;
    int mask_nbins = LASS_NBINS;
    float* pool_out = nullptr;
    long pool_bs = 0;
    int pool_h = 2;
    int gx = 0, gy = 0;
    int xcd_map = 0;
};

inline bool lass_wino4_narrow(int H, int W) { return W % 32 == 16 && H % 32 == 0; }
struct Wino4Split {
    int n = 1;
    float* part = nullptr;
};

enum ConvKind { CONV1_ACT = 0, CONV2_IDENT = 1, CONV2_SHORTCUT = 2, TCONV_ACT = 3, CONV1_ACT_PRE = 4, CONV2_IDENT_PRE = 5 };

hipError_t lass_launch_conv(ConvKind kind, const ConvArgs& p, hipStream_t stream);

bool lass_wino_supported(const ConvArgs& p);
hipError_t lass_launch_wino(ConvKind kind, const ConvArgs& p, hipStream_t stream);
hipError_t lass_launch_wino_weights(const float* w, int Cout, int Cin, float* U, hipStream_t stream);
hipError_t lass_launch_wino_shortcut_weights(const float* w, int Cout, int Cin, float* U, hipStream_t stream);

bool lass_wino4_supported(ConvKind kind, const ConvArgs& p, const Wino4Split& sk = Wino4Split());
hipError_t lass_launch_wino4(ConvKind kind, const ConvArgs& p, hipStream_t stream, const Wino4Split& sk = Wino4Split());
hipError_t lass_launch_wino4_weights(const float* w, int Cout, int Cin, float* U, hipStream_t stream);

bool lass_pw_gemm_supported(ConvKind kind, const ConvArgs& p);
hipError_t lass_launch_pw_gemm(ConvKind kind, const ConvArgs& p, hipStream_t stream);

bool lass_bf16_supported(const ConvArgs& p);
hipError_t lass_launch_conv_bf16(ConvKind kind, const ConvArgs& p, hipStream_t stream);
hipError_t lass_launch_weights_bf16(const float* w, int Cout, int Cin, int taps, void* dst, int lo, int transposed,
                                    hipStream_t stream);

bool lass_enc1_fused_bf16_supported(const ConvArgs& p, const ConvArgs& q);
hipError_t lass_launch_enc1_fused_bf16(const ConvArgs& p, const ConvArgs& q, hipStream_t stream);
bool lass_dec6_fused_bf16_supported(const ConvArgs& p, const ConvArgs& q);
hipError_t lass_launch_dec6_fused_bf16(const ConvArgs& p, const ConvArgs& q, hipStream_t stream);

bool lass_dec6u_fused_bf16_supported(const ConvArgs& p, const ConvArgs& q, const ConvArgs& u);
hipError_t lass_launch_dec6u_fused_bf16(const ConvArgs& p, const ConvArgs& q, const ConvArgs& u, hipStream_t stream);
hipError_t lass_launch_compose_up_shortcut(const float* wsc, const float* wt, int Cin, int Cup, int Ccat, int Nsc, float* out,
                                           hipStream_t stream);

hipError_t lass_launch_multi_stft(const float* wav, int B, int L, int hop, int nwin, const int* n_fft,
                                  const float2* tw2k, float* const* mag, float* const* cosv, float* const* sinv,
                                  hipStream_t stream);
struct StftBranch {
    int wlen = 0;
    float *mag = nullptr, *cosv = nullptr, *sinv = nullptr, *real = nullptr, *imag = nullptr, *x0 = nullptr;
};
hipError_t lass_launch_stft2(const float* wav, int B, int L, int n_fft, int hop, int T, int Tpad, int nbr,
                             const StftBranch* br, int magphase_sem, const float* s0, const float* h0,
                             const float2* tw2k, hipStream_t stream);
hipError_t lass_launch_istft2(const float* real, const float* imag, int B, int T, int L, int n_fft, int wlen, int hop,
                              const float2* tw2k, float* wav, hipStream_t stream);

hipError_t lass_launch_film(const float* cond, int B, const float* Wf, const float* bf, const float* base, int n,
                            float* out, hipStream_t stream);
hipError_t lass_launch_pool(const float* in, long in_bs, int B, int C, int H, int W, int ph, int pw, float* out,
                            hipStream_t stream);
hipError_t lass_launch_mask(const float* x12, const float* wa, const float* ba, const float* mag, const float* cosv,
                            const float* sinv, int B, int T, int Tpad, int fcrop, float* out_real, float* out_imag,
                            hipStream_t stream);
hipError_t lass_launch_x0_from_mag(const float* mag, int B, int T, int Tpad, int fcrop, const float* s0,
                                   const float* h0, float* x0, hipStream_t stream);
hipError_t lass_launch_sdr(const float* ref, const float* est, int B, int L, double* stats, hipStream_t stream);
hipError_t lass_launch_mix_at_snr(float* source, const float* noise, const float* snr_db, float* mixture, int B, int L,
                                  double* ws, hipStream_t stream);
hipError_t lass_launch_segment_mix(const float* waveforms, int B, int L, const int* mix_num, const float* comp_db, int max_comp,
                                   const float* noise_db, float* mixture, float* segment, double* ws, hipStream_t stream);
hipError_t lass_launch_relayout_conv(const float* src, int Cout, int Cin, int taps, float* dst, hipStream_t stream);
hipError_t lass_launch_bnfold(const float* g, const float* beta, const float* mean, const float* var, int C, float eps,
                              float* scale, float* base, hipStream_t stream);

size_t lass_resample_table_floats(int up, int n_taps);
hipError_t lass_launch_decode_resample(const void* raw, long long row_stride, int B, int frames, int ch, int enc, int up, int down,
                                       const float* taps, int n_taps, float* out, int L_out, hipStream_t stream);
```

### lass_amd/csrc/wino4.hip

```cpp
#include <hip/hip_runtime.h>
#include "kernels.h"
#include "pixel_ops.h"
#include "wino_common.h"

namespace {

constexpr int F_PRO = 1, F_PHASEB = 2, F_BIAS = 4, F_RES = 8, F_EPIACT = 16, F_PRECONV = 64, F_RESPRE = 128, F_MASK = 1024;
constexpr int F_SPLITK = 2048;
constexpr int NTHREADS = 256;
constexpr int KC = 8;
constexpr int NXI = 36;
constexpr int U_F = NXI * 256;
constexpr int V_F = NXI * 4 * 32 * 2;

typedef float f32x2v __attribute__((ext_vector_type(2)));

__device__ __forceinline__ void bt6(const float (&d)[6], float (&r)[6]) {
    const float t0 = fmaf(-4.f, d[2], d[4]);
    const float t1 = fmaf(-4.f, d[1], d[3]);
    const float t2 = d[4] - d[2];
    const float u = d[3] - d[1];
    r[0] = fmaf(4.f, d[0], fmaf(-5.f, d[2], d[4]));
    r[1] = t0 + t1;
    r[2] = t0 - t1;
    r[3] = fmaf(2.f, u, t2);
    r[4] = fmaf(-2.f, u, t2);
    r[5] = fmaf(4.f, d[1], fmaf(-5.f, d[3], d[5]));
}

__device__ __forceinline__ void at6(const float (&m)[6], float (&y)[4]) {
    const float s12 = m[1] + m[2], d12 = m[1] - m[2], s34 = m[3] + m[4], d34 = m[3] - m[4];
    y[0] = m[0] + s12 + s34;
    y[1] = fmaf(2.f, d34, d12);
    y[2] = fmaf(4.f, s34, s12);
    y[3] = fmaf(8.f, d34, d12) + m[5];
}

template <int TC, int FLAGS>
__global__ __launch_bounds__(NTHREADS, 2) void wino4_kernel(ConvArgs p) {
    const Wino4Split sk;
#include "wino4_body.h"
}
template <int TC, int FLAGS0>
__global__ __launch_bounds__(NTHREADS, 2) void wino4_splitk_kernel(ConvArgs p, Wino4Split sk) {
    constexpr int FLAGS = FLAGS0 | F_SPLITK;
#include "wino4_body.h"
}

template <int FLAGS>
__global__ __launch_bounds__(256) void wino4_combine_kernel(ConvArgs p, Wino4Split sk) {
    constexpr bool EPI = (FLAGS & F_EPIACT) != 0, RES = (FLAGS & F_RES) != 0;
    static_assert(EPI != RES && (FLAGS & ~(F_EPIACT | F_RES)) == 0, "conv1 or the identity conv2");
    const int W4 = p.W / 4, H2 = p.H / 2, HW = p.H * p.W;
    const long idx = (long)blockIdx.x * 256 + threadIdx.x;
    if (idx >= (long)p.B * p.N * H2 * W4) return;
    const int xq = (int)(idx % W4), yh = (int)(idx / W4 % H2), n = (int)(idx / ((long)W4 * H2) % p.N), b = (int)(idx / ((long)W4 * H2 * p.N));
    const size_t pix = (size_t)(2 * yh) * p.W + 4 * xq;
    const size_t split_pitch = (size_t)p.B * p.N * HW;
    const float* pp = sk.part + ((size_t)b * p.N + n) * HW + pix;
    float4 v[2];
#pragma unroll
    for (int i = 0; i < 2; ++i) v[i] = *reinterpret_cast<const float4*>(pp + (size_t)i * p.W);
    for (int s = 1; s < sk.n; ++s)
#pragma unroll
        for (int i = 0; i < 2; ++i) {
            const float4 t = *reinterpret_cast<const float4*>(pp + (size_t)s * split_pitch + (size_t)i * p.W);
            v[i].x += t.x; v[i].y += t.y; v[i].z += t.z; v[i].w += t.w;
        }
    if (EPI) {
        const float es = p.epi_scale[n], eh = p.epi_shift[(size_t)b * p.epi_shift_bs + n];
#pragma unroll
        for (int i = 0; i < 2; ++i) {
            v[i].x = leaky(fmaf(v[i].x, es, eh)); v[i].y = leaky(fmaf(v[i].y, es, eh));
            v[i].z = leaky(fmaf(v[i].z, es, eh)); v[i].w = leaky(fmaf(v[i].w, es, eh));
        }
    }
    if (RES) {
        const float* rr = p.res + (size_t)b * p.res_bs + (size_t)n * HW + pix;
        float4 t[2];
#pragma unroll
        for (int i = 0; i < 2; ++i) t[i] = *reinterpret_cast<const float4*>(rr + (size_t)i * p.W);
#pragma unroll
        for (int i = 0; i < 2; ++i) { v[i].x += t[i].x; v[i].y += t[i].y; v[i].z += t[i].z; v[i].w += t[i].w; }
    }
    float* dst = p.out + (size_t)b * p.out_bs + (size_t)n * HW + pix;
#pragma unroll
    for (int i = 0; i < 2; ++i) *reinterpret_cast<float4*>(dst + (size_t)i * p.W) = v[i];
    if (RES && p.pool_out) {
        const int Wo = p.W / 2, Ho = p.H / p.pool_h;
        float* pd = p.pool_out + (size_t)b * (p.pool_bs ? (size_t)p.pool_bs : (size_t)p.N * Ho * Wo) + (size_t)n * Ho * Wo + 2 * xq;
        if (p.pool_h == 2) {
            float s0 = v[0].x + v[0].y, s1 = v[0].z + v[0].w;
            s0 += v[1].x; s0 += v[1].y;
            s1 += v[1].z; s1 += v[1].w;
            *reinterpret_cast<float2*>(pd + (size_t)yh * Wo) = make_float2(s0 * 0.25f, s1 * 0.25f);
        } else {
#pragma unroll
            for (int i = 0; i < 2; ++i)
                *reinterpret_cast<float2*>(pd + (size_t)(2 * yh + i) * Wo) = make_float2((v[i].x + v[i].y) * 0.5f, (v[i].z + v[i].w) * 0.5f);
        }
    }
}

__global__ __launch_bounds__(256) void wino4_weights_kernel(const float* __restrict__ w, int Cout, int Cin, float* __restrict__ U) {
    const long i = (long)blockIdx.x * 256 + threadIdx.x;
    if (i >= (long)Cout * Cin) return;
    const int co = (int)(i % Cout), ci = (int)(i / Cout);
    const float* g = w + ((size_t)co * Cin + ci) * 9;
    const double G[6][3] = {{0.25, 0, 0},           {-1.0 / 6, -1.0 / 6, -1.0 / 6}, {-1.0 / 6, 1.0 / 6, -1.0 / 6},
                            {1.0 / 24, 1.0 / 12, 1.0 / 6}, {1.0 / 24, -1.0 / 12, 1.0 / 6},  {0, 0, 1}};
    double t[6][3];
    for (int a = 0; a < 6; ++a)
        for (int c = 0; c < 3; ++c) t[a][c] = G[a][0] * (double)g[0 * 3 + c] + G[a][1] * (double)g[1 * 3 + c] + G[a][2] * (double)g[2 * 3 + c];
    float* slab = U + ((size_t)(ci / 8) * (Cout / 32) + co / 32) * U_F;
    const int e = (((co & 31) >> 4) * 4 + (ci & 3)) * 32 + (co & 15) * 2 + ((ci & 7) >> 2);
    for (int a = 0; a < 6; ++a)
        for (int c = 0; c < 6; ++c) {
            const double u = t[a][0] * G[c][0] + t[a][1] * G[c][1] + t[a][2] * G[c][2];
            slab[(a * 6 + c) * 256 + e] = (float)u;
        }
}

template <int TC, int FLAGS>
hipError_t launch_wino4_tc(const ConvArgs& p0, hipStream_t stream) {
    ConvArgs p = p0;
    constexpr int OR_ = 4 * (32 / TC), OC = 4 * TC;
    p.gx = (p.W / OC) * ((p.H + OR_ - 1) / OR_);
    p.gy = p.N / 32;
    p.xcd_map = ((long)p.gx * p.B) % 8 == 0;
    hipLaunchKernelGGL((wino4_kernel<TC, FLAGS>), dim3((unsigned)((long)p.gx * p.gy * p.B)), dim3(NTHREADS), 0, stream, p);
    return hipGetLastError();
}

template <int FLAGS>
hipError_t launch_wino4(const ConvArgs& p, hipStream_t stream) {
    if (p.W % 64 == 0 && p.H % 8 == 0) return launch_wino4_tc<16, FLAGS>(p, stream);
    if (p.W % 32 == 0 && p.H % 16 == 0) return launch_wino4_tc<8, FLAGS>(p, stream);
    if constexpr (FLAGS == (F_PRO | F_EPIACT) || FLAGS == F_RES)
        if (lass_wino4_narrow(p.H, p.W)) return launch_wino4_tc<4, FLAGS>(p, stream);
    return hipErrorInvalidValue;
}

template <int MAIN, int COMB>
hipError_t launch_wino4_split(const ConvArgs& p0, const Wino4Split& sk, hipStream_t stream) {
    ConvArgs p = p0;
    p.gx = (p.W / 16) * (p.H / 32);
    p.gy = p.N / 32;
    p.xcd_map = ((long)p.gx * p.B * sk.n) % 8 == 0;
    hipLaunchKernelGGL((wino4_splitk_kernel<4, MAIN>), dim3((unsigned)((long)p.gx * p.gy * p.B * sk.n)), dim3(NTHREADS), 0, stream, p, sk);
    if (hipError_t e = hipGetLastError()) return e;
    const long items = (long)p.B * p.N * (p.H / 2) * (p.W / 4);
    hipLaunchKernelGGL((wino4_combine_kernel<COMB>), dim3((unsigned)((items + 255) / 256)), dim3(256), 0, stream, p, sk);
    return hipGetLastError();
}

}

bool lass_wino4_supported(ConvKind kind, const ConvArgs& p, const Wino4Split& sk) {
    const bool narrow = lass_wino4_narrow(p.H, p.W);
    if (!(p.w_wino4 && ((p.W % 64 == 0 && p.H % 8 == 0) || (p.W % 32 == 0 && p.H % 16 == 0) || narrow) && p.Cin % KC == 0 && p.N % 32 == 0 &&
          p.Nw % 32 == 0 && (unsigned long long)p.Cin * p.H * p.W * 4ull < 0xFFFF0000ull))
        return false;
    if (narrow) {
        if (sk.n != 1 && !(sk.n >= 2 && sk.n <= p.Cin / KC && sk.part && p.N == p.Nw)) return false;
        return kind == CONV1_ACT || (kind == CONV2_IDENT && p.res && !p.mask_re && (!p.pool_out || p.pool_h == 2 || p.pool_h == 1));
    }
    if (sk.n != 1) return false;
    switch (kind) {
        case CONV1_ACT:
            return true;
        case CONV1_ACT_PRE:
            return p.pre_w && p.pre_b && p.Cin == 32;
        case CONV2_IDENT_PRE:
            return p.res && p.pre_w && p.pre_b && p.N == 32 && p.Nw == 32 && (!p.pool_out || p.pool_h == 2);
        case CONV2_IDENT:
            return p.res && !p.mask_re && (!p.pool_out || p.pool_h == 2);
        case CONV2_SHORTCUT:
            if (!(p.in2 && p.w2 && p.bias && p.Cin2 % 16 == 0 && (!p.pool_out || p.pool_h == 2))) return false;
            if (p.mask_re)
                return p.N == 32 && p.Nw == 32 && p.W + 1 == p.mask_nbins && p.mask_w && p.mask_b && p.mask_mag && p.mask_cos && p.mask_sin &&
                       p.mask_im && p.mask_T > 0 && p.mask_T <= p.H && !p.pool_out;
            return true;
        default:
            return false;
    }
}

hipError_t lass_launch_wino4(ConvKind kind, const ConvArgs& p, hipStream_t stream, const Wino4Split& sk) {
    if (!lass_wino4_supported(kind, p, sk) || !p.in || (!p.out && !p.mask_re)) return hipErrorInvalidValue;
    switch (kind) {
        case CONV1_ACT:
        case CONV1_ACT_PRE:
            if (!p.pro_scale || !p.pro_shift || !p.epi_scale || !p.epi_shift) return hipErrorInvalidValue;
            if (sk.n > 1) return launch_wino4_split<F_PRO, F_EPIACT>(p, sk, stream);
            return kind == CONV1_ACT ? launch_wino4<F_PRO | F_EPIACT>(p, stream) : launch_wino4<F_PRO | F_EPIACT | F_PRECONV>(p, stream);
        case CONV2_IDENT:
            if (sk.n > 1) return launch_wino4_split<0, F_RES>(p, sk, stream);
            return launch_wino4<F_RES>(p, stream);
        case CONV2_IDENT_PRE:
            return launch_wino4<F_RES | F_RESPRE>(p, stream);
        case CONV2_SHORTCUT:
            return p.mask_re ? launch_wino4<F_PHASEB | F_BIAS | F_MASK>(p, stream) : launch_wino4<F_PHASEB | F_BIAS>(p, stream);
        default:
            return hipErrorInvalidValue;
    }
}

hipError_t lass_launch_wino4_weights(const float* w, int Cout, int Cin, float* U, hipStream_t stream) {
    const long n = (long)Cout * Cin;
    hipLaunchKernelGGL(wino4_weights_kernel, dim3((unsigned)((n + 255) / 256)), dim3(256), 0, stream, w, Cout, Cin, U);
    return hipGetLastError();
}
```

### lass_amd/csrc/wino4_body.h

```cpp
    constexpr bool PRO = (FLAGS & F_PRO) != 0, EPI = (FLAGS & F_EPIACT) != 0, SC = (FLAGS & F_PHASEB) != 0;
    constexpr bool PRE = (FLAGS & F_PRECONV) != 0;
    constexpr bool RESPRE = (FLAGS & F_RESPRE) != 0;
    constexpr bool MASK = (FLAGS & F_MASK) != 0;
    constexpr bool RES = (FLAGS & F_RES) != 0;
    static_assert(!SC || (FLAGS & F_BIAS) != 0, "the shortcut conv has a bias");
    static_assert(!PRE || PRO, "pre_conv is folded into the prologue's affine");
    static_assert(!RESPRE || ((FLAGS & F_RES) != 0 && !SC && !EPI), "conv2 with the identity residual");
    static_assert(!MASK || SC, "the output head sits behind decoder_block6's conv2 + shortcut");
    static_assert(!RES || (!SC && !EPI), "conv2 with a residual in place of the fused shortcut");
    constexpr bool SPLIT = (FLAGS & F_SPLITK) != 0;
    static_assert(!SPLIT || (FLAGS & ~(F_SPLITK | F_PRO)) == 0, "a split launch has a prologue at most");
    constexpr int TR = 32 / TC;
    constexpr int OR_ = 4 * TR, OC = 4 * TC;
    constexpr int NCO = 32;
    __shared__ __attribute__((aligned(16))) float lds[U_F + V_F + 2 * NCO + (MASK ? 100 : 0)];
    float* lu = lds;
    float* lv = lds + U_F;
    float* lds_es = lv + V_F;
    float* lds_eh = lds_es + NCO;
    float* lds_mw = lds_eh + NCO;

    const int tid = threadIdx.x;
    const int lane = tid & 63, wave = __builtin_amdgcn_readfirstlane(tid >> 6);
    const int wco = wave >> 1, wwt = wave & 1;
    int bx_, by_, b, ks = 0;
    if constexpr (SPLIT) {
        const unsigned lin = blockIdx.x, ngrp = (unsigned)(p.gx * p.B * sk.n);
        unsigned grp;
        if (p.xcd_map) {
            const unsigned j = lin >> 3;
            grp = (lin & 7u) * (ngrp >> 3) + j / (unsigned)p.gy;
            by_ = (int)(j % (unsigned)p.gy);
        } else {
            grp = lin / (unsigned)p.gy;
            by_ = (int)(lin % (unsigned)p.gy);
        }
        ks = (int)(grp % (unsigned)sk.n);
        const unsigned xz = grp / (unsigned)sk.n;
        b = (int)(xz / (unsigned)p.gx);
        bx_ = (int)(xz % (unsigned)p.gx);
    } else {
        block_coords(p, bx_, by_, b);
    }
    const int n0 = by_ * NCO;
    const int tiles_x = p.W / OC;
    const int y0 = (bx_ / tiles_x) * OR_, x0 = (bx_ % tiles_x) * OC;
    const int HW = p.H * p.W;
    const float* in_b = p.in + (size_t)b * p.in_bs;
    const float* sc = PRO ? p.pro_scale : nullptr;
    const float* sh = PRO ? p.pro_shift + (size_t)b * p.pro_shift_bs : nullptr;

    if (EPI && tid < NCO) {
        lds_es[tid] = p.epi_scale[n0 + tid];
        lds_eh[tid] = p.epi_shift[(size_t)b * p.epi_shift_bs + n0 + tid];
    }
    if (SC && tid < NCO) lds_es[tid] = p.bias[n0 + tid];
    if (RESPRE && tid < 32) {
        lds_es[tid] = p.pre_w[n0 + tid];
        lds_eh[tid] = p.pre_b[n0 + tid];
    }
    if (MASK && tid < 99) lds_mw[tid] = tid < 96 ? p.mask_w[tid] : p.mask_b[tid - 96];

    f32x4 acc[NXI];
#pragma unroll
    for (int xi = 0; xi < NXI; ++xi)
#pragma unroll
        for (int r = 0; r < 4; ++r) acc[xi][r] = 0.f;

    const int kq = lane >> 4, l15 = lane & 15;
    const float* afrag = lu + (wco >> 1) * U_F + (wco & 1) * 128 + (kq * 16 + l15) * 2;
    const float* bfrag = lv + (kq * 32 + ((wwt * 16 + l15) ^ ((kq & 1) << 4))) * 2;
    const unsigned slab_pitch = (unsigned)(p.Nw / 32) * (unsigned)(U_F * 4);
    const unsigned slab_n0 = (unsigned)(n0 / 32) * (unsigned)(U_F * 4);
    const unsigned lu_addr = (unsigned)(size_t)(__attribute__((address_space(3))) float*)lu;
    const unsigned ulane = (unsigned)lane * 16u;
    const v4i32 uw = make_rsrc_words(p.w_wino4, (unsigned)(NXI * p.Cin * p.Nw) * 4u);

    const int pt = tid & 31, c8 = (tid & 255) >> 5;
    const int pty = pt / TC, ptx = pt % TC;
    const int gy0 = y0 + 4 * pty - 1, gx0 = x0 + 4 * ptx - 1;
    const bool left = gx0 < 0, right = gx0 + 5 >= p.W;
    unsigned vo_c[6], vo_l[6], vo_r[6], rowok = 0;
#pragma unroll
    for (int i = 0; i < 6; ++i) {
        const int gy = gy0 + i;
        const int row = (PRE ? 0 : c8 * HW) + min(max(gy, 0), p.H - 1) * p.W;
        vo_c[i] = 4u * (unsigned)(row + gx0 + 1);
        vo_l[i] = 4u * (unsigned)(row + (left ? 0 : gx0));
        vo_r[i] = 4u * (unsigned)(row + (right ? p.W - 1 : gx0 + 5));
        rowok |= (gy >= 0 && gy < p.H ? 1u : 0u) << i;
    }
    const __amdgpu_buffer_rsrc_t in_rsrc =
        __builtin_amdgcn_make_buffer_rsrc(const_cast<float*>(in_b), 0, (int)((unsigned)(PRE ? 1 : p.Cin) * (unsigned)HW * 4u), 0x00020000);
    const bool edge = left || right || rowok != 0x3fu;
    float4 pc[6];
    float pl[6], pr[6], ps = 1.f, ph = 0.f;
    const unsigned tvo = (unsigned)c8 * 4u;
    const auto tab_rsrc = [&](const float* t, int n) {
        return __builtin_amdgcn_make_buffer_rsrc(const_cast<float*>(t), 0, n * 4, 0x00020000);
    };
    const __amdgpu_buffer_rsrc_t sc_rsrc = tab_rsrc(PRO ? sc : p.in, p.Cin), sh_rsrc = tab_rsrc(PRO ? sh : p.in, p.Cin);
    const __amdgpu_buffer_rsrc_t pw_rsrc = tab_rsrc(PRE ? p.pre_w : p.in, 32), pb_rsrc = tab_rsrc(PRE ? p.pre_b : p.in, 32);
    auto pload = [&](int ch) {
        const unsigned soff = PRE ? 0u : (unsigned)(ch * KC * HW) * 4u;
        if (!PRE || ch == 0)
#pragma unroll
        for (int i = 0; i < 6; ++i) {
            pc[i] = __builtin_bit_cast(float4, __builtin_amdgcn_raw_buffer_load_b128(in_rsrc, (int)vo_c[i], (int)soff, 0));
            pl[i] = __builtin_bit_cast(float, __builtin_amdgcn_raw_buffer_load_b32(in_rsrc, (int)vo_l[i], (int)soff, 0));
            pr[i] = __builtin_bit_cast(float, __builtin_amdgcn_raw_buffer_load_b32(in_rsrc, (int)vo_r[i], (int)soff, 0));
        }
        const unsigned toff = (unsigned)(ch * KC) * 4u;
        if (PRO) {
            ps = __builtin_bit_cast(float, __builtin_amdgcn_raw_buffer_load_b32(sc_rsrc, (int)tvo, (int)toff, 0));
            ph = __builtin_bit_cast(float, __builtin_amdgcn_raw_buffer_load_b32(sh_rsrc, (int)tvo, (int)toff, 0));
        }
        if (PRE) {
            const float pw = __builtin_bit_cast(float, __builtin_amdgcn_raw_buffer_load_b32(pw_rsrc, (int)tvo, (int)toff, 0));
            const float pb = __builtin_bit_cast(float, __builtin_amdgcn_raw_buffer_load_b32(pb_rsrc, (int)tvo, (int)toff, 0));
            ph = fmaf(pb, ps, ph);
            ps = pw * ps;
        }
    };
    constexpr int NLOAD = (PRE ? 0 : 6 * 3) + (PRO ? 2 : 0) + (PRE ? 2 : 0);
    float* vdst = lv + ((c8 & 3) * 32 + (pt ^ ((c8 & 1) << 4))) * 2 + (c8 >> 2);
    auto pprocess = [&]() {
        float d[6][6];
#pragma unroll
        for (int i = 0; i < 6; ++i) {
            const float v[6] = {pl[i], pc[i].x, pc[i].y, pc[i].z, pc[i].w, pr[i]};
#pragma unroll
            for (int jx = 0; jx < 6; ++jx) d[i][jx] = PRO ? leaky(fmaf(v[jx], ps, ph)) : v[jx];
        }
        if (__builtin_amdgcn_ballot_w64(edge) != 0) {
            const bool r0 = (rowok & 1u) != 0, r5 = (rowok & 32u) != 0;
#pragma unroll
            for (int jx = 0; jx < 6; ++jx) {
                d[0][jx] = r0 ? d[0][jx] : 0.f;
                d[5][jx] = r5 ? d[5][jx] : 0.f;
            }
#pragma unroll
            for (int i = 0; i < 6; ++i) {
                d[i][0] = left ? 0.f : d[i][0];
                d[i][5] = right ? 0.f : d[i][5];
            }
        }
        float tt[6][6];
#pragma unroll
        for (int jx = 0; jx < 6; ++jx) {
            const float col[6] = {d[0][jx], d[1][jx], d[2][jx], d[3][jx], d[4][jx], d[5][jx]};
            float r[6];
            bt6(col, r);
#pragma unroll
            for (int i = 0; i < 6; ++i) tt[i][jx] = r[i];
        }
#pragma unroll
        for (int i = 0; i < 6; ++i) {
            float r[6];
            bt6(tt[i], r);
#pragma unroll
            for (int jx = 0; jx < 6; ++jx) vdst[(i * 6 + jx) * 256] = r[jx];
        }
    };

    const int ch0 = SPLIT ? ks * (p.Cin / KC) / sk.n : 0;
    const int nch = SPLIT ? (ks + 1) * (p.Cin / KC) / sk.n : p.Cin / KC;
    pload(ch0);
    lds_barrier();
    for (int ch = ch0; ch < nch; ++ch) {
        lds_barrier();
        __builtin_amdgcn_s_setprio(2);
#pragma unroll
        for (int i = 0; i < 6; ++i) {
            asm volatile("" : "+v"(pc[i].x), "+v"(pc[i].y), "+v"(pc[i].z), "+v"(pc[i].w), "+v"(pl[i]), "+v"(pr[i]));
        }
        if (PRO) asm volatile("" : "+v"(ps), "+v"(ph));
#pragma unroll
        for (int i = 0; i < 9; ++i) {
            const unsigned piece = (unsigned)(wave * 9 + i) * 1024u;
            lds_dma_16B(uw, ulane, (unsigned)ch * slab_pitch + slab_n0 + piece, lu_addr + piece);
        }
        __builtin_amdgcn_sched_barrier(0);
        pprocess();
        __builtin_amdgcn_sched_barrier(0);
        const bool pf = ch + 1 < nch;
        if (pf) pload(ch + 1);
        __builtin_amdgcn_sched_barrier(0);
        if (pf)
            wait_vmcnt<NLOAD>();
        else
            wait_vmcnt<0>();
        lds_barrier();
        __builtin_amdgcn_s_setprio(0);
        constexpr int PFD = 2;
        f32x2v av[PFD + 1][2], bv[PFD + 1][2];
        auto rd = [&](int s) {
#pragma unroll
            for (int q = 0; q < 2; ++q) {
                av[s % (PFD + 1)][q] = *reinterpret_cast<const f32x2v*>(afrag + (2 * s + q) * 256);
                bv[s % (PFD + 1)][q] = *reinterpret_cast<const f32x2v*>(bfrag + (2 * s + q) * 256);
            }
        };
#pragma unroll
        for (int s = 0; s < PFD; ++s) rd(s);
#pragma unroll
        for (int s = 0; s < NXI / 2; ++s) {
            if (s + PFD < NXI / 2) rd(s + PFD);
            __builtin_amdgcn_sched_barrier(0);
            const f32x2v a0 = av[s % (PFD + 1)][0], a1 = av[s % (PFD + 1)][1];
            const f32x2v b0 = bv[s % (PFD + 1)][0], b1 = bv[s % (PFD + 1)][1];
            acc[2 * s] = __builtin_amdgcn_mfma_f32_16x16x4f32(a0.x, b0.x, acc[2 * s], 0, 0, 0);
            acc[2 * s + 1] = __builtin_amdgcn_mfma_f32_16x16x4f32(a1.x, b1.x, acc[2 * s + 1], 0, 0, 0);
            acc[2 * s] = __builtin_amdgcn_mfma_f32_16x16x4f32(a0.y, b0.y, acc[2 * s], 0, 0, 0);
            acc[2 * s + 1] = __builtin_amdgcn_mfma_f32_16x16x4f32(a1.y, b1.y, acc[2 * s + 1], 0, 0, 0);
            __builtin_amdgcn_sched_barrier(0);
        }
    }

    const int ot = wwt * 16 + l15;
    const int oy = y0 + 4 * (ot / TC), ox = x0 + 4 * (ot % TC);
    f32x4 ysp[16];
#pragma unroll
    for (int r = 0; r < 4; ++r) {
        const int nl = wco * 16 + kq * 4 + r;
        float tmp[4][6];
#pragma unroll
        for (int jx = 0; jx < 6; ++jx) {
            const float m[6] = {acc[0 + jx][r], acc[6 + jx][r], acc[12 + jx][r], acc[18 + jx][r], acc[24 + jx][r], acc[30 + jx][r]};
            float y[4];
            at6(m, y);
#pragma unroll
            for (int a = 0; a < 4; ++a) tmp[a][jx] = y[a];
        }
        const float es = (EPI || SC) ? lds_es[nl] : 0.f, eh = EPI ? lds_eh[nl] : 0.f;
#pragma unroll
        for (int a = 0; a < 4; ++a) {
            float y[4];
            at6(tmp[a], y);
#pragma unroll
            for (int c = 0; c < 4; ++c) {
                float v = y[c];
                if (EPI) v = leaky(fmaf(v, es, eh));
                if (SC) v += es;
                ysp[a * 4 + c][r] = v;
            }
        }
    }
    if constexpr (SPLIT) {
#pragma unroll
        for (int r = 0; r < 4; ++r) {
            const int n = n0 + wco * 16 + kq * 4 + r;
            float* dst = sk.part + (((size_t)ks * p.B + b) * p.N + n) * HW + (size_t)oy * p.W + ox;
#pragma unroll
            for (int a = 0; a < 4; ++a) {
                const float4 o = make_float4(ysp[a * 4 + 0][r], ysp[a * 4 + 1][r], ysp[a * 4 + 2][r], ysp[a * 4 + 3][r]);
                if (oy + a < p.H) *reinterpret_cast<float4*>(dst + (size_t)a * p.W) = o;
            }
        }
        return;
    }
    if constexpr (RESPRE) {
        const float* xr = p.res + (size_t)b * p.res_bs + (size_t)min(oy, p.H - 4) * p.W + ox;
        float4 xv[4];
#pragma unroll
        for (int a = 0; a < 4; ++a) xv[a] = *reinterpret_cast<const float4*>(xr + (size_t)a * p.W);
#pragma unroll
        for (int r = 0; r < 4; ++r) {
            const float pw = lds_es[wco * 16 + kq * 4 + r], pb = lds_eh[wco * 16 + kq * 4 + r];
#pragma unroll
            for (int a = 0; a < 4; ++a) {
                ysp[a * 4 + 0][r] += fmaf(xv[a].x, pw, pb);
                ysp[a * 4 + 1][r] += fmaf(xv[a].y, pw, pb);
                ysp[a * 4 + 2][r] += fmaf(xv[a].z, pw, pb);
                ysp[a * 4 + 3][r] += fmaf(xv[a].w, pw, pb);
            }
        }
    }
    if constexpr (RES && !RESPRE) {
        float4 rv[4][4];
#pragma unroll
        for (int r = 0; r < 4; ++r) {
            const float* rr = p.res + (size_t)b * p.res_bs + (size_t)(n0 + wco * 16 + kq * 4 + r) * HW + (size_t)min(oy, p.H - 4) * p.W + ox;
#pragma unroll
            for (int a = 0; a < 4; ++a) rv[r][a] = *reinterpret_cast<const float4*>(rr + (size_t)a * p.W);
        }
#pragma unroll
        for (int r = 0; r < 4; ++r)
#pragma unroll
            for (int a = 0; a < 4; ++a) {
                ysp[a * 4 + 0][r] += rv[r][a].x;
                ysp[a * 4 + 1][r] += rv[r][a].y;
                ysp[a * 4 + 2][r] += rv[r][a].z;
                ysp[a * 4 + 3][r] += rv[r][a].w;
            }
    }
    if constexpr (SC) {
        const float* x2 = p.in2 + (size_t)b * p.in2_bs + (size_t)min(oy, p.H - 4) * p.W + ox;
        const float* wsc = p.w2 + n0 + wco * 16 + l15;
        const int nks = p.Cin2 / 4;
        constexpr int NSB = 4;
        float4 xb[NSB][4];
        float wa[NSB];
        auto ldk = [&](int ks, int buf) {
            const float* xp = x2 + (size_t)(4 * ks + kq) * HW;
#pragma unroll
            for (int a = 0; a < 4; ++a) xb[buf][a] = *reinterpret_cast<const float4*>(xp + (size_t)a * p.W);
            wa[buf] = wsc[(size_t)(4 * ks + kq) * p.Nw];
        };
        auto mmk = [&](int buf) {
#pragma unroll
            for (int a = 0; a < 4; ++a) {
                ysp[a * 4 + 0] = __builtin_amdgcn_mfma_f32_16x16x4f32(wa[buf], xb[buf][a].x, ysp[a * 4 + 0], 0, 0, 0);
                ysp[a * 4 + 1] = __builtin_amdgcn_mfma_f32_16x16x4f32(wa[buf], xb[buf][a].y, ysp[a * 4 + 1], 0, 0, 0);
                ysp[a * 4 + 2] = __builtin_amdgcn_mfma_f32_16x16x4f32(wa[buf], xb[buf][a].z, ysp[a * 4 + 2], 0, 0, 0);
                ysp[a * 4 + 3] = __builtin_amdgcn_mfma_f32_16x16x4f32(wa[buf], xb[buf][a].w, ysp[a * 4 + 3], 0, 0, 0);
            }
        };
        ldk(0, 0);
        ldk(1, 1);
        ldk(2, 2);
        for (int ks = 0; ks < nks; ks += NSB) {
#pragma unroll
            for (int u = 0; u < NSB; ++u) {
                ldk(min(ks + u + 3, nks - 1), (u + 3) % NSB);
                __builtin_amdgcn_sched_barrier(0);
                mmk(u);
                __builtin_amdgcn_sched_barrier(0);
            }
        }
    }
    if constexpr (MASK) {
        float* part = lds;
        lds_barrier();
#pragma unroll
        for (int q = 0; q < 3; ++q) {
            float w4[4];
#pragma unroll
            for (int r = 0; r < 4; ++r) w4[r] = lds_mw[q * 32 + wco * 16 + kq * 4 + r];
#pragma unroll
            for (int a = 0; a < 4; ++a) {
                float4 o;
                float* op = &o.x;
#pragma unroll
                for (int c = 0; c < 4; ++c) {
                    const f32x4 v = ysp[a * 4 + c];
                    op[c] = v[0] * w4[0] + v[1] * w4[1] + v[2] * w4[2] + v[3] * w4[3];
                }
                *reinterpret_cast<float4*>(part + ((wco * 4 + kq) * 3 + q) * 512 + ot * 16 + a * 4) = o;
            }
        }
        lds_barrier();
        const int px = tid * 2;
        const int mt = px >> 4, ms = px & 15;
        const int my = y0 + 4 * (mt / TC) + (ms >> 2), mx = x0 + 4 * (mt % TC) + (ms & 3);
        float lg[3][2];
#pragma unroll
        for (int q = 0; q < 3; ++q) {
            float2 sum = make_float2(lds_mw[96 + q], lds_mw[96 + q]);
#pragma unroll
            for (int src = 0; src < 8; ++src) {
                const float2 v = *reinterpret_cast<const float2*>(part + (src * 3 + q) * 512 + px);
                sum.x += v.x;
                sum.y += v.y;
            }
            lg[q][0] = sum.x;
            lg[q][1] = sum.y;
        }
        if (my < p.mask_T) {
            mask_pixel(p, b, my, mx, lg[0][0], lg[1][0], lg[2][0]);
            mask_pixel(p, b, my, mx + 1, lg[0][1], lg[1][1], lg[2][1]);
        }
        return;
    }
#pragma unroll
    for (int r = 0; r < 4; ++r) {
        const int n = n0 + wco * 16 + kq * 4 + r;
        float* dst = p.out + (size_t)b * p.out_bs + (size_t)n * HW + (size_t)oy * p.W + ox;
#pragma unroll
        for (int a = 0; a < 4; ++a) {
            const float4 o = make_float4(ysp[a * 4 + 0][r], ysp[a * 4 + 1][r], ysp[a * 4 + 2][r], ysp[a * 4 + 3][r]);
            if (oy + a < p.H) *reinterpret_cast<float4*>(dst + (size_t)a * p.W) = o;
        }
        if constexpr (TC == 4 && RES) {
            if (p.pool_out && p.pool_h == 1) {
                const int Wo = p.W / 2;
                float* pd = p.pool_out + (size_t)b * (p.pool_bs ? (size_t)p.pool_bs : (size_t)p.N * p.H * Wo) + (size_t)n * p.H * Wo +
                            (size_t)oy * Wo + (ox >> 1);
#pragma unroll
                for (int a = 0; a < 4; ++a) {
                    float2 o;
                    o.x = (ysp[a * 4 + 0][r] + ysp[a * 4 + 1][r]) * 0.5f;
                    o.y = (ysp[a * 4 + 2][r] + ysp[a * 4 + 3][r]) * 0.5f;
                    if (oy + a < p.H) *reinterpret_cast<float2*>(pd + (size_t)a * Wo) = o;
                }
                continue;
            }
        }
        if ((SC || RES) && p.pool_out) {
            const int Ho = p.H / 2, Wo = p.W / 2;
            float* pd = p.pool_out + (size_t)b * (p.pool_bs ? (size_t)p.pool_bs : (size_t)p.N * Ho * Wo) + (size_t)n * Ho * Wo +
                        (size_t)(oy >> 1) * Wo + (ox >> 1);
#pragma unroll
            for (int i = 0; i < 2; ++i) {
                float2 o;
                float s0 = ysp[(2 * i) * 4 + 0][r] + ysp[(2 * i) * 4 + 1][r];
                s0 += ysp[(2 * i + 1) * 4 + 0][r];
                s0 += ysp[(2 * i + 1) * 4 + 1][r];
                float s1 = ysp[(2 * i) * 4 + 2][r] + ysp[(2 * i) * 4 + 3][r];
                s1 += ysp[(2 * i + 1) * 4 + 2][r];
                s1 += ysp[(2 * i + 1) * 4 + 3][r];
                o.x = s0 * 0.25f;
                o.y = s1 * 0.25f;
                if (oy + 2 * i + 1 < p.H) *reinterpret_cast<float2*>(pd + (size_t)i * Wo) = o;
            }
        }
    }
```

Before: 1030 clips/s.

## Precompute Winograd F(4,3) input transform into memory for wide-Cout convs

Adds a separate prep kernel that computes the Winograd input-tile transform (with optional prologue activation) once per input chunk and writes it to a workspace image. The main wino4 kernel then DMAs the pre-transformed V tiles straight into LDS instead of loading and transforming the input itself. This applies to layers with many output-channel groups, where the same input transform was otherwise recomputed by every Cout block. The cost is an extra launch, extra workspace memory and extra global write/read traffic for the V image.

```diff
diff --git a/include/lass_hip.h b/include/lass_hip.h
--- a/include/lass_hip.h
+++ b/include/lass_hip.h
@@ -44,6 +44,8 @@
 int lass_graph_stats(const lass_ctx* ctx, long* captures, long* replays);
 int lass_set_graph_replay(lass_ctx* ctx, int enabled);
 int lass_set_wino4_splits(lass_ctx* ctx, int splits);
+int lass_set_wino4_vprep(lass_ctx* ctx, int mode);
+int lass_set_wino4_vprep_buffer(lass_ctx* ctx, float* v, size_t floats);
 
 int lass_separate_components(lass_ctx* ctx, const float* const* mag, const float* cos_mask, const float* sin_mask,
                              const float* condition, float* out, int B, int L, void* workspace, size_t workspace_bytes,
diff --git a/lass_amd/_lib.py b/lass_amd/_lib.py
--- a/lass_amd/_lib.py
+++ b/lass_amd/_lib.py
@@ -31,6 +31,8 @@
     ("lass_graph_stats", c_int, [c_void_p, POINTER(c_long), POINTER(c_long)]),
     ("lass_set_graph_replay", c_int, [c_void_p, c_int]),
     ("lass_set_wino4_splits", c_int, [c_void_p, c_int]),
+    ("lass_set_wino4_vprep", c_int, [c_void_p, c_int]),
+    ("lass_set_wino4_vprep_buffer", c_int, [c_void_p, c_void_p, c_size_t]),
     ("lass_separate_components", c_int, [c_void_p, POINTER(c_void_p), c_void_p, c_void_p, c_void_p, c_void_p, c_int,
                                          c_int, c_void_p, c_size_t, c_void_p]),
     ("lass_stft_components", c_int, [c_void_p, c_void_p, c_int, c_int, c_int, c_int, c_int, POINTER(c_int),
diff --git a/lass_amd/csrc/api.hip b/lass_amd/csrc/api.hip
--- a/lass_amd/csrc/api.hip
+++ b/lass_amd/csrc/api.hip
@@ -96,6 +96,11 @@
     int compute_mode = LASS_COMPUTE_F32;
     int wino4_mincin = 32;
     int ksplit_force = 0;
+    int vprep_mode = 1;
+    float* stage_v = nullptr;
+    size_t stage_v_floats = 0;
+    float* stage_v_user = nullptr;
+    size_t stage_v_user_floats = 0;
     float* stage_part = nullptr;
     size_t stage_part_floats = 0;
     bool fuse_catb = true;
@@ -400,6 +405,8 @@
     const CatCopies* pool_copies = nullptr;
     const UpFuse* up = nullptr;
     float* kpart = nullptr;
+    float* vws = nullptr;
+    size_t vws_floats = 0;
 };
 
 constexpr int kWino4Splits = 4;
@@ -412,6 +419,20 @@
 size_t wino4_split_floats(const ResBlock& rb, int S, int B, int H, int W) { return S > 1 ? (size_t)S * B * rb.cout * H * W : 0; }
 
 constexpr int kShortcutGemmMinCin = 256;
+
+constexpr int kVprepMinCoutGroups = 12;
+bool wino4_level_geom(const ResBlock& rb, int H, int W, int ksplit) { return rb.width % 32 == 0 ? !lass_wino4_narrow(H, W) : ksplit > 0; }
+bool wino4_vprep_shape(const lass_ctx* c, const ResBlock& rb) {
+    if (c->compute_mode != LASS_COMPUTE_F32 || c->vprep_mode == 0 || c->wino4_mincin <= 0) return false;
+    return c->vprep_mode == 2 || rb.cout / 32 >= kVprepMinCoutGroups;
+}
+size_t wino4_vprep_floats(const lass_ctx* c, const ResBlock& rb, int B, int H, int W) {
+    if (!wino4_vprep_shape(c, rb) || rb.cin % 8 != 0 || rb.cout % 32 != 0) return 0;
+    if (!lass_wino4_block_tc(H, W) || !wino4_level_geom(rb, H, W, wino4_splits(c, rb, B, H, W))) return 0;
+    int ch = rb.u1f ? rb.cin : 0;
+    if (rb.u2f && (rb.cin == rb.cout || rb.cin >= kShortcutGemmMinCin)) ch = std::max(ch, rb.cout);
+    return lass_wino4_vpre_floats(B, ch, H, W);
+}
 
 int run_resblock(lass_ctx* c, const ResBlock& rb, const float* x, long x_bs, int B, int H, int W, const float* shift,
                  float* a2, float* out, long out_bs, hipStream_t st, const BlockFusions& f = BlockFusions()) {
@@ -443,7 +464,7 @@
     const ConvKind k1 = x0 ? CONV1_ACT_PRE : CONV1_ACT, k2 = x0 ? CONV2_IDENT_PRE : CONV2_IDENT;
     const bool wino1 = !bf1 && rb.u1 && lass_wino_supported(p);
     const int ksplit = bf1 || x0 ? 0 : wino4_splits(c, rb, B, H, W);
-    const bool w4_geom = rb.width % 32 == 0 ? !lass_wino4_narrow(H, W) : ksplit > 0;
+    const bool w4_geom = wino4_level_geom(rb, H, W, ksplit);
     if (ksplit > 1) {
         if (!f.kpart) return fail(c, LASS_ERR_STATE, "split-K needs its partial workspace");
         const auto overlaps = [&](const float* a, size_t a_n, const float* b, long b_bs, long b_n) {
@@ -456,12 +477,32 @@
     }
     Wino4Split sk;
     if (ksplit > 1) { sk.n = ksplit; sk.part = f.kpart; }
+    const size_t vneed = !bf1 && !x0 && w4_geom ? wino4_vprep_floats(c, rb, B, H, W) : 0;
+    if (vneed) {
+        if (!f.vws || f.vws_floats < vneed) return fail(c, LASS_ERR_STATE, "the V-from-memory route needs its image workspace");
+        const auto overlaps = [&](const float* b, long b_bs, long b_n) {
+            return b && f.vws < b + (size_t)(B - 1) * b_bs + b_n && b < f.vws + vneed;
+        };
+        if (overlaps(x, x_bs, rb.cin * HW) || overlaps(a2, rb.cout * HW, rb.cout * HW) || overlaps(out, out_bs, rb.cout * HW) ||
+            (sk.part && overlaps(sk.part, 0, (long)wino4_split_floats(rb, ksplit, B, H, W))))
+            return fail(c, LASS_ERR_STATE, "the V image must not overlap the block's input, intermediate, output or split-K partials");
+    }
+    auto vprep_slot = [&](int cin, Wino4VPre* vp) -> int {
+        if (lass_wino4_vpre_floats(B, cin, H, W) > vneed) return fail(c, LASS_ERR_STATE, "the V image workspace is smaller than this layer's image");
+        vp->v = f.vws;
+        return 0;
+    };
+    const bool vshape = vneed > 0;
     auto launch_conv1 = [&]() -> int {
         ProfScope ps(c, st, P_CONV3X3);
         if (bf1)
             HIP_TRY(c, lass_launch_conv_bf16(k1, p, st));
-        else if (wino1 && rb.u1f && w4_geom && lass_wino4_supported(k1, p, sk))
-            HIP_TRY(c, lass_launch_wino4(k1, p, st, sk));
+        else if (wino1 && rb.u1f && w4_geom && lass_wino4_supported(k1, p, sk)) {
+            Wino4VPre vp;
+            if (vshape && lass_wino4_vpre_supported(k1, p, sk))
+                if (int rv = vprep_slot(rb.cin, &vp)) return rv;
+            HIP_TRY(c, lass_launch_wino4(k1, p, st, sk, vp));
+        }
         else if (wino1)
             HIP_TRY(c, lass_launch_wino(k1, p, st));
         else
@@ -552,12 +593,19 @@
         r.in2 = nullptr; r.in2_bs = 0; r.Cin2 = 0; r.w2 = nullptr; r.bias = nullptr;
         r.res = out; r.res_bs = out_bs;
         if (!lass_wino4_supported(CONV2_IDENT, r, sk)) return fail(c, LASS_ERR_STATE, "conv2 with the shortcut as residual");
-        HIP_TRY(c, lass_launch_wino4(CONV2_IDENT, r, st, sk));
+        Wino4VPre vp;
+        if (vshape && lass_wino4_vpre_supported(CONV2_IDENT, r, sk))
+            if (int rv = vprep_slot(rb.cout, &vp)) return rv;
+        HIP_TRY(c, lass_launch_wino4(CONV2_IDENT, r, st, sk, vp));
     } else if (rb.cin == rb.cout) {
         if (bf2)
             HIP_TRY(c, lass_launch_conv_bf16(k2, q, st));
-        else if (wino2 && (x0 || ksplit > 0) && q.w_wino4 && lass_wino4_supported(k2, q, sk))
-            HIP_TRY(c, lass_launch_wino4(k2, q, st, sk));
+        else if (wino2 && (x0 || ksplit > 0) && q.w_wino4 && lass_wino4_supported(k2, q, sk)) {
+            Wino4VPre vp;
+            if (vshape && lass_wino4_vpre_supported(k2, q, sk))
+                if (int rv = vprep_slot(rb.cout, &vp)) return rv;
+            HIP_TRY(c, lass_launch_wino4(k2, q, st, sk, vp));
+        }
         else if (wino2)
             HIP_TRY(c, lass_launch_wino(k2, q, st));
         else
@@ -616,6 +664,7 @@
     size_t mag, cosv, sinv, x0[kMaxBranches], shift, a2, cat[6], pool[6], center, decout[6], oreal, oimag;
     size_t kpart = 0;
     bool has_kpart = false;
+    size_t vprep = 0, vprep_floats = 0;
     int eh[7], ew[7];
 };
 
@@ -657,17 +706,21 @@
     }
     pl->a2 = bump(t, a2max);
     pl->oreal = bump(t, spec); pl->oimag = bump(t, spec);
-    size_t kmax = 0;
+    size_t kmax = 0, vmax = 0;
     for (int i = 1; i < 7; ++i) {
         const ResBlock& rb = trunk_block(c, i);
+        vmax = std::max(vmax, wino4_vprep_floats(c, rb, B, pl->eh[i], pl->ew[i]));
         kmax = std::max(kmax, wino4_split_floats(rb, wino4_splits(c, rb, B, pl->eh[i], pl->ew[i]), B, pl->eh[i], pl->ew[i]));
     }
     for (int d = 0; d < 6; ++d) {
         const ResBlock& rb = c->dec[d];
+        vmax = std::max(vmax, wino4_vprep_floats(c, rb, B, pl->eh[5 - d], pl->ew[5 - d]));
         kmax = std::max(kmax, wino4_split_floats(rb, wino4_splits(c, rb, B, pl->eh[5 - d], pl->ew[5 - d]), B, pl->eh[5 - d], pl->ew[5 - d]));
     }
     pl->has_kpart = kmax > 0;
     if (kmax) pl->kpart = bump(t, kmax);
+    pl->vprep_floats = vmax;
+    if (vmax) pl->vprep = bump(t, vmax);
     return 0;
 }
 
@@ -694,7 +747,7 @@
 
 bool split_halves(const lass_ctx* c, int B) { return c->split_batch > 0 && !c->profiling && B >= 8 && (B % 2) == 0; }
 
-int stage_kpart(lass_ctx* c, const ResBlock& rb, int B, int H, int W, BlockFusions* f) {
+int stage_scratch(lass_ctx* c, const ResBlock& rb, int B, int H, int W, BlockFusions* f) {
     const size_t need = wino4_split_floats(rb, wino4_splits(c, rb, B, H, W), B, H, W);
     if (need > c->stage_part_floats) {
         if (c->stage_part) HIP_TRY(c, hipFree(c->stage_part));
@@ -704,6 +757,19 @@
         c->stage_part_floats = need;
     }
     if (need) f->kpart = c->stage_part;
+    const size_t vneed = wino4_vprep_floats(c, rb, B, H, W);
+    if (c->stage_v_user) {
+        if (vneed) { f->vws = c->stage_v_user; f->vws_floats = c->stage_v_user_floats; }
+        return 0;
+    }
+    if (vneed > c->stage_v_floats) {
+        if (c->stage_v) HIP_TRY(c, hipFree(c->stage_v));
+        c->stage_v = nullptr;
+        c->stage_v_floats = 0;
+        HIP_TRY(c, hipMalloc((void**)&c->stage_v, vneed * sizeof(float)));
+        c->stage_v_floats = vneed;
+    }
+    if (vneed) { f->vws = c->stage_v; f->vws_floats = c->stage_v_floats; }
     return 0;
 }
 
@@ -752,6 +818,7 @@
     if (const char* e = getenv("LASS_FUSE_BLOCK")) c->fuse_block = atoi(e) != 0;
     if (const char* e = getenv("LASS_FUSE_UP")) c->fuse_up = atoi(e) != 0;
     if (const char* e = getenv("LASS_WINO4")) c->wino4_mincin = atoi(e);
+    if (const char* e = getenv("LASS_WINO4_VPREP")) c->vprep_mode = std::max(0, std::min(2, atoi(e)));
     if (const char* e = getenv("LASS_SPLIT")) c->split_batch = std::max(0, std::min(2, atoi(e)));
     if (const char* e = getenv("LASS_GRAPH")) c->use_graph = atoi(e) != 0;
     c->prof.resize(P_COUNT);
@@ -826,6 +893,7 @@
     if (c->ev_fork) (void)hipEventDestroy(c->ev_fork);
     (void)hipFree(c->tw2k);
     (void)hipFree(c->stage_part);
+    (void)hipFree(c->stage_v);
     delete c;
     return 0;
 }
@@ -1129,7 +1197,7 @@
     if (!rb) return fail(c, LASS_ERR_ARG, std::string("lass_convblock: unknown block '") + prefix + "'");
     const long HW = (long)H * W;
     BlockFusions f;
-    if ((r = stage_kpart(c, *rb, B, H, W, &f))) return r;
+    if ((r = stage_scratch(c, *rb, B, H, W, &f))) return r;
     return run_resblock(c, *rb, x, rb->cin * HW, B, H, W, shift, scratch, y, rb->cout * HW, (hipStream_t)stream, f);
 }
 
@@ -1150,7 +1218,7 @@
         hipStream_t st = (hipStream_t)stream;
         BlockFusions f;
         if (fuse) { f.pool_out = pool; f.pool_h = e.dh; }
-        if ((r = stage_kpart(c, rb, B, H, W, &f))) return r;
+        if ((r = stage_scratch(c, rb, B, H, W, &f))) return r;
         r = run_resblock(c, rb, x, rb.cin * HW, B, H, W, shift, scratch, y, rb.cout * HW, st, f);
         if (r) return r;
         if (pooled && !fuse) HIP_TRY(c, lass_launch_pool(y, rb.cout * HW, B, rb.cout, H, W, e.dh, e.dw, pool, st));
@@ -1417,6 +1485,7 @@
             if (i >= 1 && i <= 4 && use_pc[i - 1]) f.cat_in = &pc[i - 1];
             if (i < 4 && use_pc[i]) f.pool_copies = &pc[i];
             if (pl.has_kpart) f.kpart = F(pl.kpart);
+            if (pl.vprep_floats) { f.vws = F(pl.vprep); f.vws_floats = pl.vprep_floats; }
             r = run_resblock(c, rb, x, rb.cin * HW, B, H, W, shift, F(pl.a2), o, o_bs, st, f);
             if (r) return r;
         }
@@ -1447,6 +1516,7 @@
         const MaskHead head{mag_m, cos_m, sin_m, F(pl.oreal), F(pl.oimag), T, g.nbins};
         if (d == 5) f.head = &head;
         if (pl.has_kpart) f.kpart = F(pl.kpart);
+        if (pl.vprep_floats) { f.vws = F(pl.vprep); f.vws_floats = pl.vprep_floats; }
         r = run_resblock(c, rb, F(pl.cat[d]), rb.cin * HW, B, H, W, shift, F(pl.a2), F(pl.decout[d]), rb.cout * HW, st, f);
         if (r) return r;
         x = F(pl.decout[d]);
@@ -1579,6 +1649,20 @@
     return 0;
 }
 
+int lass_set_wino4_vprep(lass_ctx* c, int mode) {
+    if (!c || mode < 0 || mode > 2) return fail(c, LASS_ERR_ARG, "lass_set_wino4_vprep: 0, 1 or 2");
+    c->vprep_mode = mode;
+    ++c->gen;
+    return 0;
+}
+
+int lass_set_wino4_vprep_buffer(lass_ctx* c, float* v, size_t floats) {
+    if (!c || (v && !floats)) return fail(c, LASS_ERR_ARG, "lass_set_wino4_vprep_buffer: a buffer and its size, or NULL");
+    c->stage_v_user = v;
+    c->stage_v_user_floats = v ? floats : 0;
+    return 0;
+}
+
 int lass_graph_stats(const lass_ctx* c, long* captures, long* replays) {
     if (!c) return LASS_ERR_ARG;
     if (captures) *captures = c->g_captures;
diff --git a/lass_amd/csrc/kernels.h b/lass_amd/csrc/kernels.h
--- a/lass_amd/csrc/kernels.h
+++ b/lass_amd/csrc/kernels.h
@@ -77,9 +77,18 @@
 };
 
 inline bool lass_wino4_narrow(int H, int W) { return W % 32 == 16 && H % 32 == 0; }
+inline int lass_wino4_block_tc(int H, int W) {
+    if (W % 64 == 0 && H % 8 == 0) return 16;
+    if (W % 32 == 0 && H % 16 == 0) return 8;
+    return lass_wino4_narrow(H, W) ? 4 : 0;
+}
 struct Wino4Split {
     int n = 1;
     float* part = nullptr;
+};
+
+struct Wino4VPre {
+    float* v = nullptr;
 };
 
 enum ConvKind { CONV1_ACT = 0, CONV2_IDENT = 1, CONV2_SHORTCUT = 2, TCONV_ACT = 3, CONV1_ACT_PRE = 4, CONV2_IDENT_PRE = 5 };
@@ -92,7 +101,10 @@
 hipError_t lass_launch_wino_shortcut_weights(const float* w, int Cout, int Cin, float* U, hipStream_t stream);
 
 bool lass_wino4_supported(ConvKind kind, const ConvArgs& p, const Wino4Split& sk = Wino4Split());
-hipError_t lass_launch_wino4(ConvKind kind, const ConvArgs& p, hipStream_t stream, const Wino4Split& sk = Wino4Split());
+hipError_t lass_launch_wino4(ConvKind kind, const ConvArgs& p, hipStream_t stream, const Wino4Split& sk = Wino4Split(),
+                             const Wino4VPre& vp = Wino4VPre());
+bool lass_wino4_vpre_supported(ConvKind kind, const ConvArgs& p, const Wino4Split& sk = Wino4Split());
+size_t lass_wino4_vpre_floats(int B, int Cin, int H, int W);
 hipError_t lass_launch_wino4_weights(const float* w, int Cout, int Cin, float* U, hipStream_t stream);
 
 bool lass_pw_gemm_supported(ConvKind kind, const ConvArgs& p);
diff --git a/lass_amd/csrc/wino4.hip b/lass_amd/csrc/wino4.hip
--- a/lass_amd/csrc/wino4.hip
+++ b/lass_amd/csrc/wino4.hip
@@ -7,6 +7,7 @@
 
 constexpr int F_PRO = 1, F_PHASEB = 2, F_BIAS = 4, F_RES = 8, F_EPIACT = 16, F_PRECONV = 64, F_RESPRE = 128, F_MASK = 1024;
 constexpr int F_SPLITK = 2048;
+constexpr int F_VPRE = 4096;
 constexpr int NTHREADS = 256;
 constexpr int KC = 8;
 constexpr int NXI = 36;
@@ -39,12 +40,47 @@
 template <int TC, int FLAGS>
 __global__ __launch_bounds__(NTHREADS, 2) void wino4_kernel(ConvArgs p) {
     const Wino4Split sk;
+    const Wino4VPre vp;
 #include "wino4_body.h"
 }
 template <int TC, int FLAGS0>
 __global__ __launch_bounds__(NTHREADS, 2) void wino4_splitk_kernel(ConvArgs p, Wino4Split sk) {
     constexpr int FLAGS = FLAGS0 | F_SPLITK;
+    const Wino4VPre vp;
 #include "wino4_body.h"
+}
+template <int TC, int FLAGS0>
+__global__ __launch_bounds__(NTHREADS, 2) void wino4_vpre_kernel(ConvArgs p, Wino4Split sk, Wino4VPre vp) {
+    constexpr int FLAGS = FLAGS0 | F_VPRE;
+#include "wino4_body.h"
+}
+
+template <int TC, int FLAGS>
+__global__ __launch_bounds__(NTHREADS) void wino4_vprep_kernel(ConvArgs p, Wino4VPre vp) {
+    constexpr bool PRO = (FLAGS & F_PRO) != 0, PRE = false;
+    static_assert((FLAGS & ~F_PRO) == 0, "a prologue at most");
+    constexpr int TR = 32 / TC;
+    constexpr int OR_ = 4 * TR, OC = 4 * TC;
+    __shared__ __attribute__((aligned(16))) float lv[V_F];
+    const int tid = threadIdx.x;
+    const unsigned nchunk = (unsigned)(p.Cin / KC);
+    const unsigned lin = blockIdx.x;
+    const int ch = (int)(lin % nchunk);
+    const int bx_ = (int)(lin / nchunk % (unsigned)p.gx), b = (int)(lin / nchunk / (unsigned)p.gx);
+    const int tiles_x = p.W / OC;
+    const int y0 = (bx_ / tiles_x) * OR_, x0 = (bx_ % tiles_x) * OC;
+    const int HW = p.H * p.W;
+    const float* in_b = p.in + (size_t)b * p.in_bs;
+    const float* sc = PRO ? p.pro_scale : nullptr;
+    const float* sh = PRO ? p.pro_shift + (size_t)b * p.pro_shift_bs : nullptr;
+#include "wino4_input.h"
+    pload(ch);
+    pprocess();
+    __syncthreads();
+    float4* dst = reinterpret_cast<float4*>(vp.v + (((size_t)b * p.gx + bx_) * nchunk + ch) * V_F);
+    const float4* src = reinterpret_cast<const float4*>(lv);
+#pragma unroll
+    for (int i = 0; i < V_F / 4 / NTHREADS; ++i) dst[i * NTHREADS + tid] = src[i * NTHREADS + tid];
 }
 
 template <int FLAGS>
@@ -134,10 +170,49 @@
 
 template <int FLAGS>
 hipError_t launch_wino4(const ConvArgs& p, hipStream_t stream) {
-    if (p.W % 64 == 0 && p.H % 8 == 0) return launch_wino4_tc<16, FLAGS>(p, stream);
-    if (p.W % 32 == 0 && p.H % 16 == 0) return launch_wino4_tc<8, FLAGS>(p, stream);
+    const int tc = lass_wino4_block_tc(p.H, p.W);
+    if (tc == 16) return launch_wino4_tc<16, FLAGS>(p, stream);
+    if (tc == 8) return launch_wino4_tc<8, FLAGS>(p, stream);
     if constexpr (FLAGS == (F_PRO | F_EPIACT) || FLAGS == F_RES)
-        if (lass_wino4_narrow(p.H, p.W)) return launch_wino4_tc<4, FLAGS>(p, stream);
+        if (tc == 4) return launch_wino4_tc<4, FLAGS>(p, stream);
+    return hipErrorInvalidValue;
+}
+
+template <int TC, int MAIN, int COMB>
+hipError_t launch_wino4_vpre_tc(const ConvArgs& p0, const Wino4Split& sk, const Wino4VPre& vp, bool pro, hipStream_t stream) {
+    ConvArgs p = p0;
+    constexpr int OR_ = 4 * (32 / TC), OC = 4 * TC;
+    constexpr bool SPLIT = (MAIN & F_SPLITK) != 0;
+    const int n = SPLIT ? sk.n : 1;
+    p.gx = (p.W / OC) * (p.H / OR_);
+    p.gy = p.N / 32;
+    p.xcd_map = ((long)p.gx * p.B * n) % 8 == 0;
+    const dim3 pgrid((unsigned)((long)p.gx * (p.Cin / KC) * p.B));
+    if (pro)
+        hipLaunchKernelGGL((wino4_vprep_kernel<TC, F_PRO>), pgrid, dim3(NTHREADS), 0, stream, p, vp);
+    else
+        hipLaunchKernelGGL((wino4_vprep_kernel<TC, 0>), pgrid, dim3(NTHREADS), 0, stream, p, vp);
+    if (hipError_t e = hipGetLastError()) return e;
+    Wino4Split s1 = sk;
+    if (!SPLIT) s1 = Wino4Split();
+    hipLaunchKernelGGL((wino4_vpre_kernel<TC, MAIN>), dim3((unsigned)((long)p.gx * p.gy * p.B * n)), dim3(NTHREADS), 0, stream, p, s1, vp);
+    if (hipError_t e = hipGetLastError()) return e;
+    if constexpr (SPLIT) {
+        const long items = (long)p.B * p.N * (p.H / 2) * (p.W / 4);
+        hipLaunchKernelGGL((wino4_combine_kernel<COMB>), dim3((unsigned)((items + 255) / 256)), dim3(256), 0, stream, p, sk);
+        return hipGetLastError();
+    }
+    return hipSuccess;
+}
+
+template <int EPI>
+hipError_t launch_wino4_vpre(const ConvArgs& p, const Wino4Split& sk, const Wino4VPre& vp, hipStream_t stream) {
+    constexpr bool pro = EPI == F_EPIACT;
+    const int tc = lass_wino4_block_tc(p.H, p.W);
+    if (tc == 16) return launch_wino4_vpre_tc<16, EPI, 0>(p, sk, vp, pro, stream);
+    if (tc == 8) return launch_wino4_vpre_tc<8, EPI, 0>(p, sk, vp, pro, stream);
+    if (tc == 4)
+        return sk.n > 1 ? launch_wino4_vpre_tc<4, F_SPLITK, EPI>(p, sk, vp, pro, stream) : launch_wino4_vpre_tc<4, EPI, 0>(p, sk, vp, pro, stream);
     return hipErrorInvalidValue;
 }
 
@@ -157,8 +232,8 @@
 }
 
 bool lass_wino4_supported(ConvKind kind, const ConvArgs& p, const Wino4Split& sk) {
-    const bool narrow = lass_wino4_narrow(p.H, p.W);
-    if (!(p.w_wino4 && ((p.W % 64 == 0 && p.H % 8 == 0) || (p.W % 32 == 0 && p.H % 16 == 0) || narrow) && p.Cin % KC == 0 && p.N % 32 == 0 &&
+    const bool narrow = lass_wino4_block_tc(p.H, p.W) == 4;
+    if (!(p.w_wino4 && lass_wino4_block_tc(p.H, p.W) != 0 && p.Cin % KC == 0 && p.N % 32 == 0 &&
           p.Nw % 32 == 0 && (unsigned long long)p.Cin * p.H * p.W * 4ull < 0xFFFF0000ull))
         return false;
     if (narrow) {
@@ -186,8 +261,23 @@
     }
 }
 
-hipError_t lass_launch_wino4(ConvKind kind, const ConvArgs& p, hipStream_t stream, const Wino4Split& sk) {
+size_t lass_wino4_vpre_floats(int B, int Cin, int H, int W) { return (size_t)B * Cin * (size_t)(H * W / 16) * NXI; }
+
+bool lass_wino4_vpre_supported(ConvKind kind, const ConvArgs& p, const Wino4Split& sk) {
+    return (kind == CONV1_ACT || kind == CONV2_IDENT) && lass_wino4_supported(kind, p, sk) && !p.mask_re &&
+           (unsigned long long)(p.Cin / KC) * V_F * 4ull < 0xFFFF0000ull;
+}
+
+hipError_t lass_launch_wino4(ConvKind kind, const ConvArgs& p, hipStream_t stream, const Wino4Split& sk, const Wino4VPre& vp) {
     if (!lass_wino4_supported(kind, p, sk) || !p.in || (!p.out && !p.mask_re)) return hipErrorInvalidValue;
+    if (vp.v) {
+        if (!lass_wino4_vpre_supported(kind, p, sk)) return hipErrorInvalidValue;
+        if (kind == CONV1_ACT) {
+            if (!p.pro_scale || !p.pro_shift || !p.epi_scale || !p.epi_shift) return hipErrorInvalidValue;
+            return launch_wino4_vpre<F_EPIACT>(p, sk, vp, stream);
+        }
+        return launch_wino4_vpre<F_RES>(p, sk, vp, stream);
+    }
     switch (kind) {
         case CONV1_ACT:
         case CONV1_ACT_PRE:
diff --git a/lass_amd/csrc/wino4_body.h b/lass_amd/csrc/wino4_body.h
--- a/lass_amd/csrc/wino4_body.h
+++ b/lass_amd/csrc/wino4_body.h
@@ -9,7 +9,9 @@
     static_assert(!MASK || SC, "the output head sits behind decoder_block6's conv2 + shortcut");
     static_assert(!RES || (!SC && !EPI), "conv2 with a residual in place of the fused shortcut");
     constexpr bool SPLIT = (FLAGS & F_SPLITK) != 0;
-    static_assert(!SPLIT || (FLAGS & ~(F_SPLITK | F_PRO)) == 0, "a split launch has a prologue at most");
+    static_assert(!SPLIT || (FLAGS & ~(F_SPLITK | F_PRO | F_VPRE)) == 0, "a split launch has a prologue at most");
+    constexpr bool VPRE = (FLAGS & F_VPRE) != 0;
+    static_assert(!VPRE || (FLAGS & ~(F_VPRE | F_SPLITK | F_EPIACT | F_RES)) == 0, "conv1 / identity conv2 / split share: the prologue ran in the prep launch");
     constexpr int TR = 32 / TC;
     constexpr int OR_ = 4 * TR, OC = 4 * TC;
     constexpr int NCO = 32;
@@ -76,120 +78,49 @@
     const unsigned ulane = (unsigned)lane * 16u;
     const v4i32 uw = make_rsrc_words(p.w_wino4, (unsigned)(NXI * p.Cin * p.Nw) * 4u);
 
-    const int pt = tid & 31, c8 = (tid & 255) >> 5;
-    const int pty = pt / TC, ptx = pt % TC;
-    const int gy0 = y0 + 4 * pty - 1, gx0 = x0 + 4 * ptx - 1;
-    const bool left = gx0 < 0, right = gx0 + 5 >= p.W;
-    unsigned vo_c[6], vo_l[6], vo_r[6], rowok = 0;
-#pragma unroll
-    for (int i = 0; i < 6; ++i) {
-        const int gy = gy0 + i;
-        const int row = (PRE ? 0 : c8 * HW) + min(max(gy, 0), p.H - 1) * p.W;
-        vo_c[i] = 4u * (unsigned)(row + gx0 + 1);
-        vo_l[i] = 4u * (unsigned)(row + (left ? 0 : gx0));
-        vo_r[i] = 4u * (unsigned)(row + (right ? p.W - 1 : gx0 + 5));
-        rowok |= (gy >= 0 && gy < p.H ? 1u : 0u) << i;
-    }
-    const __amdgpu_buffer_rsrc_t in_rsrc =
-        __builtin_amdgcn_make_buffer_rsrc(const_cast<float*>(in_b), 0, (int)((unsigned)(PRE ? 1 : p.Cin) * (unsigned)HW * 4u), 0x00020000);
-    const bool edge = left || right || rowok != 0x3fu;
-    float4 pc[6];
-    float pl[6], pr[6], ps = 1.f, ph = 0.f;
-    const unsigned tvo = (unsigned)c8 * 4u;
-    const auto tab_rsrc = [&](const float* t, int n) {
-        return __builtin_amdgcn_make_buffer_rsrc(const_cast<float*>(t), 0, n * 4, 0x00020000);
-    };
-    const __amdgpu_buffer_rsrc_t sc_rsrc = tab_rsrc(PRO ? sc : p.in, p.Cin), sh_rsrc = tab_rsrc(PRO ? sh : p.in, p.Cin);
-    const __amdgpu_buffer_rsrc_t pw_rsrc = tab_rsrc(PRE ? p.pre_w : p.in, 32), pb_rsrc = tab_rsrc(PRE ? p.pre_b : p.in, 32);
-    auto pload = [&](int ch) {
-        const unsigned soff = PRE ? 0u : (unsigned)(ch * KC * HW) * 4u;
-        if (!PRE || ch == 0)
-#pragma unroll
-        for (int i = 0; i < 6; ++i) {
-            pc[i] = __builtin_bit_cast(float4, __builtin_amdgcn_raw_buffer_load_b128(in_rsrc, (int)vo_c[i], (int)soff, 0));
-            pl[i] = __builtin_bit_cast(float, __builtin_amdgcn_raw_buffer_load_b32(in_rsrc, (int)vo_l[i], (int)soff, 0));
-            pr[i] = __builtin_bit_cast(float, __builtin_amdgcn_raw_buffer_load_b32(in_rsrc, (int)vo_r[i], (int)soff, 0));
-        }
-        const unsigned toff = (unsigned)(ch * KC) * 4u;
-        if (PRO) {
-            ps = __builtin_bit_cast(float, __builtin_amdgcn_raw_buffer_load_b32(sc_rsrc, (int)tvo, (int)toff, 0));
-            ph = __builtin_bit_cast(float, __builtin_amdgcn_raw_buffer_load_b32(sh_rsrc, (int)tvo, (int)toff, 0));
-        }
-        if (PRE) {
-            const float pw = __builtin_bit_cast(float, __builtin_amdgcn_raw_buffer_load_b32(pw_rsrc, (int)tvo, (int)toff, 0));
-            const float pb = __builtin_bit_cast(float, __builtin_amdgcn_raw_buffer_load_b32(pb_rsrc, (int)tvo, (int)toff, 0));
-            ph = fmaf(pb, ps, ph);
-            ps = pw * ps;
-        }
-    };
-    constexpr int NLOAD = (PRE ? 0 : 6 * 3) + (PRO ? 2 : 0) + (PRE ? 2 : 0);
-    float* vdst = lv + ((c8 & 3) * 32 + (pt ^ ((c8 & 1) << 4))) * 2 + (c8 >> 2);
-    auto pprocess = [&]() {
-        float d[6][6];
-#pragma unroll
-        for (int i = 0; i < 6; ++i) {
-            const float v[6] = {pl[i], pc[i].x, pc[i].y, pc[i].z, pc[i].w, pr[i]};
-#pragma unroll
-            for (int jx = 0; jx < 6; ++jx) d[i][jx] = PRO ? leaky(fmaf(v[jx], ps, ph)) : v[jx];
-        }
-        if (__builtin_amdgcn_ballot_w64(edge) != 0) {
-            const bool r0 = (rowok & 1u) != 0, r5 = (rowok & 32u) != 0;
-#pragma unroll
-            for (int jx = 0; jx < 6; ++jx) {
-                d[0][jx] = r0 ? d[0][jx] : 0.f;
-                d[5][jx] = r5 ? d[5][jx] : 0.f;
-            }
-#pragma unroll
-            for (int i = 0; i < 6; ++i) {
-                d[i][0] = left ? 0.f : d[i][0];
-                d[i][5] = right ? 0.f : d[i][5];
-            }
-        }
-        float tt[6][6];
-#pragma unroll
-        for (int jx = 0; jx < 6; ++jx) {
-            const float col[6] = {d[0][jx], d[1][jx], d[2][jx], d[3][jx], d[4][jx], d[5][jx]};
-            float r[6];
-            bt6(col, r);
-#pragma unroll
-            for (int i = 0; i < 6; ++i) tt[i][jx] = r[i];
-        }
-#pragma unroll
-        for (int i = 0; i < 6; ++i) {
-            float r[6];
-            bt6(tt[i], r);
-#pragma unroll
-            for (int jx = 0; jx < 6; ++jx) vdst[(i * 6 + jx) * 256] = r[jx];
-        }
-    };
+#include "wino4_input.h"
+    const unsigned lv_addr = (unsigned)(size_t)(__attribute__((address_space(3))) float*)lv;
+    const v4i32 vw = make_rsrc_words(VPRE ? vp.v + ((size_t)b * p.gx + bx_) * (size_t)(p.Cin / KC) * V_F : nullptr,
+                                     (unsigned)(p.Cin / KC) * (unsigned)(V_F * 4));
 
     const int ch0 = SPLIT ? ks * (p.Cin / KC) / sk.n : 0;
     const int nch = SPLIT ? (ks + 1) * (p.Cin / KC) / sk.n : p.Cin / KC;
-    pload(ch0);
+    if constexpr (!VPRE) pload(ch0);
     lds_barrier();
     for (int ch = ch0; ch < nch; ++ch) {
         lds_barrier();
         __builtin_amdgcn_s_setprio(2);
-#pragma unroll
-        for (int i = 0; i < 6; ++i) {
-            asm volatile("" : "+v"(pc[i].x), "+v"(pc[i].y), "+v"(pc[i].z), "+v"(pc[i].w), "+v"(pl[i]), "+v"(pr[i]));
-        }
-        if (PRO) asm volatile("" : "+v"(ps), "+v"(ph));
+        if constexpr (!VPRE) {
+#pragma unroll
+            for (int i = 0; i < 6; ++i) {
+                asm volatile("" : "+v"(pc[i].x), "+v"(pc[i].y), "+v"(pc[i].z), "+v"(pc[i].w), "+v"(pl[i]), "+v"(pr[i]));
+            }
+            if (PRO) asm volatile("" : "+v"(ps), "+v"(ph));
+        }
 #pragma unroll
         for (int i = 0; i < 9; ++i) {
             const unsigned piece = (unsigned)(wave * 9 + i) * 1024u;
             lds_dma_16B(uw, ulane, (unsigned)ch * slab_pitch + slab_n0 + piece, lu_addr + piece);
         }
-        __builtin_amdgcn_sched_barrier(0);
-        pprocess();
-        __builtin_amdgcn_sched_barrier(0);
-        const bool pf = ch + 1 < nch;
-        if (pf) pload(ch + 1);
-        __builtin_amdgcn_sched_barrier(0);
-        if (pf)
-            wait_vmcnt<NLOAD>();
-        else
+        if constexpr (VPRE) {
+#pragma unroll
+            for (int i = 0; i < 9; ++i) {
+                const unsigned piece = (unsigned)(wave * 9 + i) * 1024u;
+                lds_dma_16B(vw, ulane, (unsigned)ch * (unsigned)(V_F * 4) + piece, lv_addr + piece);
+            }
             wait_vmcnt<0>();
+        } else {
+            __builtin_amdgcn_sched_barrier(0);
+            pprocess();
+            __builtin_amdgcn_sched_barrier(0);
+            const bool pf = ch + 1 < nch;
+            if (pf) pload(ch + 1);
+            __builtin_amdgcn_sched_barrier(0);
+            if (pf)
+                wait_vmcnt<NLOAD>();
+            else
+                wait_vmcnt<0>();
+        }
         lds_barrier();
         __builtin_amdgcn_s_setprio(0);
         constexpr int PFD = 2;
diff --git a/lass_amd/csrc/wino4_input.h b/lass_amd/csrc/wino4_input.h
--- /dev/null
+++ b/lass_amd/csrc/wino4_input.h
@@ -0,0 +1,86 @@
+    const int pt = tid & 31, c8 = (tid & 255) >> 5;
+    const int pty = pt / TC, ptx = pt % TC;
+    const int gy0 = y0 + 4 * pty - 1, gx0 = x0 + 4 * ptx - 1;
+    const bool left = gx0 < 0, right = gx0 + 5 >= p.W;
+    unsigned vo_c[6], vo_l[6], vo_r[6], rowok = 0;
+#pragma unroll
+    for (int i = 0; i < 6; ++i) {
+        const int gy = gy0 + i;
+        const int row = (PRE ? 0 : c8 * HW) + min(max(gy, 0), p.H - 1) * p.W;
+        vo_c[i] = 4u * (unsigned)(row + gx0 + 1);
+        vo_l[i] = 4u * (unsigned)(row + (left ? 0 : gx0));
+        vo_r[i] = 4u * (unsigned)(row + (right ? p.W - 1 : gx0 + 5));
+        rowok |= (gy >= 0 && gy < p.H ? 1u : 0u) << i;
+    }
+    const __amdgpu_buffer_rsrc_t in_rsrc =
+        __builtin_amdgcn_make_buffer_rsrc(const_cast<float*>(in_b), 0, (int)((unsigned)(PRE ? 1 : p.Cin) * (unsigned)HW * 4u), 0x00020000);
+    const bool edge = left || right || rowok != 0x3fu;
+    float4 pc[6];
+    float pl[6], pr[6], ps = 1.f, ph = 0.f;
+    const unsigned tvo = (unsigned)c8 * 4u;
+    const auto tab_rsrc = [&](const float* t, int n) {
+        return __builtin_amdgcn_make_buffer_rsrc(const_cast<float*>(t), 0, n * 4, 0x00020000);
+    };
+    const __amdgpu_buffer_rsrc_t sc_rsrc = tab_rsrc(PRO ? sc : p.in, p.Cin), sh_rsrc = tab_rsrc(PRO ? sh : p.in, p.Cin);
+    const __amdgpu_buffer_rsrc_t pw_rsrc = tab_rsrc(PRE ? p.pre_w : p.in, 32), pb_rsrc = tab_rsrc(PRE ? p.pre_b : p.in, 32);
+    auto pload = [&](int ch) {
+        const unsigned soff = PRE ? 0u : (unsigned)(ch * KC * HW) * 4u;
+        if (!PRE || ch == 0)
+#pragma unroll
+        for (int i = 0; i < 6; ++i) {
+            pc[i] = __builtin_bit_cast(float4, __builtin_amdgcn_raw_buffer_load_b128(in_rsrc, (int)vo_c[i], (int)soff, 0));
+            pl[i] = __builtin_bit_cast(float, __builtin_amdgcn_raw_buffer_load_b32(in_rsrc, (int)vo_l[i], (int)soff, 0));
+            pr[i] = __builtin_bit_cast(float, __builtin_amdgcn_raw_buffer_load_b32(in_rsrc, (int)vo_r[i], (int)soff, 0));
+        }
+        const unsigned toff = (unsigned)(ch * KC) * 4u;
+        if (PRO) {
+            ps = __builtin_bit_cast(float, __builtin_amdgcn_raw_buffer_load_b32(sc_rsrc, (int)tvo, (int)toff, 0));
+            ph = __builtin_bit_cast(float, __builtin_amdgcn_raw_buffer_load_b32(sh_rsrc, (int)tvo, (int)toff, 0));
+        }
+        if (PRE) {
+            const float pw = __builtin_bit_cast(float, __builtin_amdgcn_raw_buffer_load_b32(pw_rsrc, (int)tvo, (int)toff, 0));
+            const float pb = __builtin_bit_cast(float, __builtin_amdgcn_raw_buffer_load_b32(pb_rsrc, (int)tvo, (int)toff, 0));
+            ph = fmaf(pb, ps, ph);
+            ps = pw * ps;
+        }
+    };
+    constexpr int NLOAD = (PRE ? 0 : 6 * 3) + (PRO ? 2 : 0) + (PRE ? 2 : 0);
+    float* vdst = lv + ((c8 & 3) * 32 + (pt ^ ((c8 & 1) << 4))) * 2 + (c8 >> 2);
+    auto pprocess = [&]() {
+        float d[6][6];
+#pragma unroll
+        for (int i = 0; i < 6; ++i) {
+            const float v[6] = {pl[i], pc[i].x, pc[i].y, pc[i].z, pc[i].w, pr[i]};
+#pragma unroll
+            for (int jx = 0; jx < 6; ++jx) d[i][jx] = PRO ? leaky(fmaf(v[jx], ps, ph)) : v[jx];
+        }
+        if (__builtin_amdgcn_ballot_w64(edge) != 0) {
+            const bool r0 = (rowok & 1u) != 0, r5 = (rowok & 32u) != 0;
+#pragma unroll
+            for (int jx = 0; jx < 6; ++jx) {
+                d[0][jx] = r0 ? d[0][jx] : 0.f;
+                d[5][jx] = r5 ? d[5][jx] : 0.f;
+            }
+#pragma unroll
+            for (int i = 0; i < 6; ++i) {
+                d[i][0] = left ? 0.f : d[i][0];
+                d[i][5] = right ? 0.f : d[i][5];
+            }
+        }
+        float tt[6][6];
+#pragma unroll
+        for (int jx = 0; jx < 6; ++jx) {
+            const float col[6] = {d[0][jx], d[1][jx], d[2][jx], d[3][jx], d[4][jx], d[5][jx]};
+            float r[6];
+            bt6(col, r);
+#pragma unroll
+            for (int i = 0; i < 6; ++i) tt[i][jx] = r[i];
+        }
+#pragma unroll
+        for (int i = 0; i < 6; ++i) {
+            float r[6];
+            bt6(tt[i], r);
+#pragma unroll
+            for (int jx = 0; jx < 6; ++jx) vdst[(i * 6 + jx) * 256] = r[jx];
+        }
+    };
```

Measured after the change: 1042 clips/s (median of 6 runs). 1.2% higher.
